# fraunhoferhhi/vvdec

Hardware: NVIDIA H100
Metric: decoded frames/sec, 4K 10-bit Main10 RA, bit-exact YUV vs reference (higher is better)
Workload: dtype int16 samples / int32 accumulate

## Files before the change

### vvdec_b200/csrc/api.cu

```cuda
#include "common.cuh"
#include <stdarg.h>
#include <string.h>
#include <mutex>

namespace b200 {

static thread_local char g_err[512] = "";

void set_error(const char* fmt, ...)
{
  va_list ap; va_start(ap, fmt);
  vsnprintf(g_err, sizeof(g_err), fmt, ap);
  va_end(ap);
}

int ensure_device()
{
  static std::once_flag once;
  static int status = 0;
  std::call_once(once, [] {
    int n = 0;
    if (cudaGetDeviceCount(&n) != cudaSuccess || n == 0) { set_error("no CUDA device: vvdec_b200 has no CPU fallback"); status = B200_ERR_NO_DEVICE; return; }
    int dev = 0; cudaGetDevice(&dev);
    cudaDeviceProp p; cudaGetDeviceProperties(&p, dev);
    if (p.major != 9 || p.minor != 0) { set_error("device %s is sm_%d%d; this library is built for sm_90a only", p.name, p.major, p.minor); status = B200_ERR_NO_DEVICE; }
  });
  if (status) set_error("no usable sm_90 device: vvdec_b200 has no CPU fallback");
  return status;
}

struct HostWrapScratch {
  DevBuf planes[3], tus, coefs, scaling, misc[8];
  cudaStream_t stream = nullptr;
  int init() { if (!stream) { B200_CUDA(cudaStreamCreateWithFlags(&stream, cudaStreamNonBlocking)); } return 0; }
};
static HostWrapScratch g_hw;
HostWrapScratch& host_scratch() { return g_hw; }

static int upload_planes(const b200_geom* g, int16_t* const planes[3], DevPlanes& dp, cudaStream_t s)
{
  const int nPlanes = g->chromaFormat ? 3 : 1;
  for (int c = 0; c < nPlanes; c++) {
    const int ph = c ? g->height >> 1 : g->height;
    const size_t bytes = (size_t)g->stride[c] * ph * sizeof(int16_t);
    if (int rc = g_hw.planes[c].reserve(bytes)) return rc;
    dp.p[c] = g_hw.planes[c].as<int16_t>(); dp.stride[c] = g->stride[c];
    B200_CUDA(cudaMemcpyAsync(dp.p[c], planes[c], bytes, cudaMemcpyHostToDevice, s));
  }
  return 0;
}
static int download_planes(const b200_geom* g, int16_t* const planes[3], const DevPlanes& dp, cudaStream_t s)
{
  const int nPlanes = g->chromaFormat ? 3 : 1;
  for (int c = 0; c < nPlanes; c++) {
    const int ph = c ? g->height >> 1 : g->height;
    B200_CUDA(cudaMemcpyAsync(planes[c], dp.p[c], (size_t)g->stride[c] * ph * sizeof(int16_t), cudaMemcpyDeviceToHost, s));
  }
  return 0;
}

int num_sms()
{
  static int cache[64] = {0};
  int dev = 0; cudaGetDevice(&dev);
  if (dev < 0 || dev >= 64) dev = 0;
  if (!cache[dev]) { int n = 0; if (cudaDeviceGetAttribute(&n, cudaDevAttrMultiProcessorCount, dev) != cudaSuccess || n <= 0) n = 132; cache[dev] = n; }
  return cache[dev];
}

int fetch_list_meta(const int* metaDev, int* cnt, int nLists, const char* what, cudaStream_t s)
{
  int h[LM_INTS];
  B200_CUDA(cudaMemcpyAsync(h, metaDev, sizeof(h), cudaMemcpyDeviceToHost, s));
  B200_CUDA(cudaStreamSynchronize(s));
  for (int i = 0; i < nLists; i++) cnt[i] = h[LM_CNT + i];
  B200_CHECK(!(h[LM_ERR] & 1), "%s: invalid record (reference slots, block size or flag combination)", what);
  B200_CHECK(!(h[LM_ERR] & 2), "%s: more tiles than the picture can hold (overlapping PUs?)", what);
  return 0;
}

}

using namespace b200;

extern "C" {

B200_API const char* b200_last_error(void) { return g_err; }
B200_API const char* b200_version(void) { return "vvdec_b200 0.1 (sm_90a)"; }
B200_API int b200_device_count(void) { int n = 0; return cudaGetDeviceCount(&n) == cudaSuccess ? n : 0; }

B200_API int b200_k1_residual(const b200_geom* g, int16_t* const planes[3], const b200_tu* tus, size_t numTus,
                              const int16_t* coefs, size_t numCoefs, const int32_t* scaling, size_t numScaling, int mode)
{
  B200_CHECK(g && planes && (tus || !numTus), "b200_k1_residual: null argument");
  B200_CHECK(g->bitDepth >= 8 && g->bitDepth <= 12, "b200_k1_residual: bit depth %d unsupported", g->bitDepth);
  if (int rc = ensure_device()) return rc;
  if (int rc = g_hw.init()) return rc;
  cudaStream_t s = g_hw.stream;
  K1Launch L; L.geom = *g; L.numTus = numTus; L.mode = mode;
  if (int rc = upload_planes(g, planes, L.planes, s)) return rc;
  if (int rc = g_hw.tus.reserve(numTus * sizeof(b200_tu))) return rc;
  if (int rc = g_hw.coefs.reserve(numCoefs * sizeof(int16_t) + 16)) return rc;
  if (int rc = g_hw.scaling.reserve(numScaling * sizeof(int32_t) + 16)) return rc;
  if (int rc = g_hw.misc[4].reserve(numTus * 4 + LM_INTS * sizeof(int) + 256)) return rc;
  if (numTus) B200_CUDA(cudaMemcpyAsync(g_hw.tus.p, tus, numTus * sizeof(b200_tu), cudaMemcpyHostToDevice, s));
  if (numCoefs) B200_CUDA(cudaMemcpyAsync(g_hw.coefs.p, coefs, numCoefs * sizeof(int16_t), cudaMemcpyHostToDevice, s));
  if (numScaling) B200_CUDA(cudaMemcpyAsync(g_hw.scaling.p, scaling, numScaling * sizeof(int32_t), cudaMemcpyHostToDevice, s));
  L.tus = g_hw.tus.as<b200_tu>(); L.coefs = g_hw.coefs.as<int16_t>(); L.scaling = g_hw.scaling.as<int32_t>();
  int* meta = g_hw.misc[4].as<int>(); uint32_t* idx = reinterpret_cast<uint32_t*>(meta + LM_INTS);
  if (int rc = launch_tu_bucket(L.tus, numTus, idx, meta, *g, numCoefs, numScaling, s)) return rc;
  L.idx = idx; L.meta = meta;
  if (int rc = fetch_list_meta(meta, L.cnt, K1_LISTS, "b200_k1_residual", s)) return rc;
  StreamSet ss(s);
  if (int rc = launch_k1_residual(L, ss)) return rc;
  if (int rc = download_planes(g, planes, L.planes, s)) return rc;
  B200_CUDA(cudaStreamSynchronize(s));
  return 0;
}

B200_API int b200_lf_deblock(const b200_geom* g, int16_t* const planes[3], const b200_lf_param* lfV, const b200_lf_param* lfH,
                             const uint8_t* ctuSlice, const b200_lf_slice* slices, int numSlices, const b200_lf_seq* seq, int dirs)
{
  B200_CHECK(g && planes && lfV && lfH && slices, "b200_lf_deblock: null argument");
  B200_CHECK(numSlices >= 1 && numSlices <= 64, "b200_lf_deblock: numSlices %d out of range 1..64", numSlices);
  B200_CHECK(g->ctuSize == 32 || g->ctuSize == 64 || g->ctuSize == 128, "b200_lf_deblock: CTU size %d", g->ctuSize);
  if (int rc = ensure_device()) return rc;
  if (int rc = g_hw.init()) return rc;
  cudaStream_t s = g_hw.stream;
  LfLaunch L; L.geom = *g; L.dirs = dirs;
  memset(&L.slices, 0, sizeof(L.slices)); memcpy(L.slices.s, slices, numSlices * sizeof(b200_lf_slice));
  if (seq) L.seq = *seq; else memset(&L.seq, 0, sizeof(L.seq));
  if (int rc = upload_planes(g, planes, L.planes, s)) return rc;
  const size_t n4 = (size_t)((g->width + 3) >> 2) * ((g->height + 3) >> 2);
  const size_t nCtu = (size_t)((g->width + g->ctuSize - 1) / g->ctuSize) * ((g->height + g->ctuSize - 1) / g->ctuSize);
  if (int rc = g_hw.misc[0].reserve(n4 * sizeof(b200_lf_param))) return rc;
  if (int rc = g_hw.misc[1].reserve(n4 * sizeof(b200_lf_param))) return rc;
  if (int rc = g_hw.misc[2].reserve(nCtu)) return rc;
  B200_CUDA(cudaMemcpyAsync(g_hw.misc[0].p, lfV, n4 * sizeof(b200_lf_param), cudaMemcpyHostToDevice, s));
  B200_CUDA(cudaMemcpyAsync(g_hw.misc[1].p, lfH, n4 * sizeof(b200_lf_param), cudaMemcpyHostToDevice, s));
  if (ctuSlice) B200_CUDA(cudaMemcpyAsync(g_hw.misc[2].p, ctuSlice, nCtu, cudaMemcpyHostToDevice, s));
  L.lfV = g_hw.misc[0].as<b200_lf_param>(); L.lfH = g_hw.misc[1].as<b200_lf_param>();
  L.ctuSlice = ctuSlice ? g_hw.misc[2].as<uint8_t>() : nullptr;
  if (int rc = launch_lf_deblock(L, s)) return rc;
  if (int rc = download_planes(g, planes, L.planes, s)) return rc;
  B200_CUDA(cudaStreamSynchronize(s));
  return 0;
}

static int upload_src_alloc_dst(const b200_geom* g, const int16_t* const src[3], DevPlanes& ds, DevPlanes& dd, cudaStream_t s)
{
  const int nPlanes = g->chromaFormat ? 3 : 1;
  for (int c = 0; c < nPlanes; c++) {
    const int ph = c ? g->height >> 1 : g->height;
    const size_t bytes = (size_t)g->stride[c] * ph * sizeof(int16_t);
    if (int rc = g_hw.planes[c].reserve(bytes)) return rc;
    if (int rc = g_hw.misc[3 + c].reserve(bytes)) return rc;
    ds.p[c] = g_hw.planes[c].as<int16_t>(); dd.p[c] = g_hw.misc[3 + c].as<int16_t>(); ds.stride[c] = dd.stride[c] = g->stride[c];
    B200_CUDA(cudaMemcpyAsync(ds.p[c], src[c], bytes, cudaMemcpyHostToDevice, s));
  }
  return 0;
}

B200_API int b200_sao_picture(const b200_geom* g, const int16_t* const src[3], int16_t* const dst[3], const b200_sao_ctu* ctus, const b200_vb* vb)
{
  B200_CHECK(g && src && dst && ctus, "b200_sao_picture: null argument");
  B200_CHECK((g->width & 7) == 0 && (g->stride[0] & 3) == 0 && (!g->chromaFormat || (g->stride[1] & 3) == 0), "b200_sao_picture: width must be a multiple of 8, strides of 4");
  if (int rc = ensure_device()) return rc;
  if (int rc = g_hw.init()) return rc;
  cudaStream_t s = g_hw.stream;
  SaoLaunch L; L.geom = *g;
  if (vb) L.vb = *vb; else memset(&L.vb, 0, sizeof(L.vb));
  if (int rc = upload_src_alloc_dst(g, src, L.src, L.dst, s)) return rc;
  const size_t nCtu = (size_t)((g->width + g->ctuSize - 1) / g->ctuSize) * ((g->height + g->ctuSize - 1) / g->ctuSize);
  if (int rc = g_hw.misc[0].reserve(nCtu * sizeof(b200_sao_ctu))) return rc;
  B200_CUDA(cudaMemcpyAsync(g_hw.misc[0].p, ctus, nCtu * sizeof(b200_sao_ctu), cudaMemcpyHostToDevice, s));
  L.ctus = g_hw.misc[0].as<b200_sao_ctu>();
  if (int rc = launch_sao(L, s)) return rc;
  if (int rc = download_planes(g, dst, L.dst, s)) return rc;
  B200_CUDA(cudaStreamSynchronize(s));
  return 0;
}

B200_API int b200_intra_reconstruct(const b200_geom* g, int16_t* const planes[3], const int16_t* const resi[3], const b200_intra_tu* tus, size_t numTus)
{
  B200_CHECK(g && planes && (tus || !numTus), "b200_intra_reconstruct: null argument");
  B200_CHECK(g->bitDepth >= 8 && g->bitDepth <= 12, "b200_intra_reconstruct: bit depth %d unsupported", g->bitDepth);
  const int nPl = g->chromaFormat ? 3 : 1;
  for (size_t i = 0; i < numTus; i++) {
    const b200_intra_tu& t = tus[i];
    const int w = 1 << t.log2w, h = 1 << t.log2h, pw = t.comp ? g->width >> 1 : g->width, ph = t.comp ? g->height >> 1 : g->height, unit = t.comp ? 2 : 4;
    const bool inCtu = intra_record_in_ctu(t, intra_ctu_log2(*g));
    if (t.flags & B200_INTRA_ISP) {
      B200_CHECK(intra_isp_record_ok(t, i ? &tus[i - 1] : nullptr, g->width, g->height), "b200_intra_reconstruct: record %zu: bad ISP region", i);
      B200_CHECK(inCtu, "b200_intra_reconstruct: intra block record %zu is not inside one CTU", i);
      continue;
    }
    B200_CHECK(t.comp < nPl && t.log2w >= 2 && t.log2w <= 6 && t.log2h >= 1 && t.log2h <= 6 && t.x + w <= pw && t.y + h <= ph && !(t.x % unit) && !(t.y % unit),
               "b200_intra_reconstruct: record %zu: bad geometry", i);
    B200_CHECK(inCtu, "b200_intra_reconstruct: intra block record %zu is not inside one CTU", i);
    B200_CHECK(t.mode <= B200_INTRA_MDLM_T && t.multiRefIdx <= 2 && (!t.multiRefIdx || !t.comp), "b200_intra_reconstruct: record %zu: bad mode / reference line", i);
    B200_CHECK(!t.ciip || (t.ciip <= 3 && t.mode == B200_INTRA_PLANAR), "b200_intra_reconstruct: record %zu: bad CIIP block", i);
    B200_CHECK(t.mode < B200_INTRA_LM || (t.comp && t.log2w <= 5 && t.log2h <= 5 && t.lmAbove <= w && t.lmLeft <= h && (!(t.flags & B200_INTRA_LM_ABOVE) || t.y >= 2) && (!(t.flags & B200_INTRA_LM_LEFT) || t.x >= 2)
                                        && t.x + std::max(w, 2 * (int)t.lmAbove) <= pw && t.y + std::max(h, 2 * (int)t.lmLeft) <= ph), "b200_intra_reconstruct: record %zu: bad CCLM block", i);
    B200_CHECK(t.mode != B200_INTRA_MIP || (!t.comp && !t.multiRefIdx && (t.mip & 0x7f) < ((w == 4 && h == 4) ? 16 : (w == 4 || h == 4 || (w == 8 && h == 8)) ? 8 : 6)),
               "b200_intra_reconstruct: record %zu: bad MIP mode", i);
    B200_CHECK(t.numAbove <= 2 * w / unit && t.numLeft <= 2 * h / unit && (!t.numAbove || t.y > t.multiRefIdx) && (!t.numLeft || t.x > t.multiRefIdx)
               && (!(t.flags & B200_INTRA_AVAIL_TL) || (t.x > t.multiRefIdx && t.y > t.multiRefIdx)) && t.x + (int)t.numAbove * unit <= pw && t.y + (int)t.numLeft * unit <= ph,
               "b200_intra_reconstruct: record %zu: availability outside the picture", i);
  }
  if (int rc = ensure_device()) return rc;
  if (int rc = g_hw.init()) return rc;
  cudaStream_t s = g_hw.stream;
  IntraLaunch L; L.geom = *g; L.numTus = numTus;
  if (int rc = upload_planes(g, planes, L.planes, s)) return rc;
  for (int c = 0; c < 3; c++) {
    L.resi[c] = nullptr; L.owner[c] = nullptr; L.ownerStride[c] = 0; L.ownerBytes[c] = 0;
    if (c >= nPl) continue;
    const int pw = c ? g->width >> 1 : g->width, ph = c ? g->height >> 1 : g->height, unit = c ? 2 : 4;
    L.ownerStride[c] = (pw + unit - 1) / unit; L.ownerBytes[c] = (size_t)L.ownerStride[c] * ((ph + unit - 1) / unit) * sizeof(int);
    if (int rc = g_hw.misc[c].reserve(L.ownerBytes[c])) return rc;
    L.owner[c] = g_hw.misc[c].as<int>();
    if (resi && resi[c]) {
      const size_t bytes = (size_t)g->stride[c] * ph * sizeof(int16_t);
      if (int rc = g_hw.misc[3 + c].reserve(bytes)) return rc;
      B200_CUDA(cudaMemcpyAsync(g_hw.misc[3 + c].p, resi[c], bytes, cudaMemcpyHostToDevice, s));
      L.resi[c] = g_hw.misc[3 + c].as<int16_t>();
    }
  }
  if (int rc = g_hw.tus.reserve(numTus * sizeof(b200_intra_tu) + 16)) return rc;
  if (int rc = g_hw.misc[6].reserve((numTus + 2) * sizeof(int))) return rc;
  if (int rc = g_hw.misc[7].reserve(intra_order_ints(*g, numTus) * sizeof(int))) return rc;
  if (numTus) B200_CUDA(cudaMemcpyAsync(g_hw.tus.p, tus, numTus * sizeof(b200_intra_tu), cudaMemcpyHostToDevice, s));
  L.tus = g_hw.tus.as<b200_intra_tu>(); L.sync = g_hw.misc[6].as<int>(); L.order = g_hw.misc[7].as<int>();
  if (int rc = launch_intra(L, s)) return rc;
  int err = 0;
  if (numTus) B200_CUDA(cudaMemcpyAsync(&err, L.sync + numTus + 1, sizeof(int), cudaMemcpyDeviceToHost, s));
  if (int rc = download_planes(g, planes, L.planes, s)) return rc;
  B200_CUDA(cudaStreamSynchronize(s));
  B200_CHECK(!(err & INTRA_ERR_CTU_BLOCKS), "b200_intra_reconstruct: a CTU holds more than %d intra block records (overlapping records?)", INTRA_MAX_CTU_BLOCKS);
  B200_CHECK(!err, "b200_intra_reconstruct: a block waited for a neighbour that never finished, or the blocks of a CTU are not contiguous (list not in decoding order?)");
  return 0;
}

B200_API int b200_intra_predict(const b200_geom* g, int16_t* const planes[3], const b200_intra_tu* tus, size_t numTus)
{
  return b200_intra_reconstruct(g, planes, nullptr, tus, numTus);
}

B200_API int b200_alf_picture(const b200_geom* g, const int16_t* const src[3], int16_t* const dst[3], const b200_alf_ctu* ctus, const b200_alf_tables* T)
{
  B200_CHECK(g && src && dst && ctus && T, "b200_alf_picture: null argument");
  B200_CHECK((g->width & 7) == 0 && (g->stride[0] & 3) == 0 && (!g->chromaFormat || (g->stride[1] & 3) == 0), "b200_alf_picture: width must be a multiple of 8, strides of 4");
  B200_CHECK(T->numLumaSets >= 16 && T->numLumaSets <= 24, "b200_alf_picture: numLumaSets %d", T->numLumaSets);
  if (int rc = ensure_device()) return rc;
  if (int rc = g_hw.init()) return rc;
  cudaStream_t s = g_hw.stream;
  AlfLaunch L; L.geom = *g;
  if (int rc = upload_src_alloc_dst(g, src, L.src, L.dst, s)) return rc;
  const size_t nCtu = (size_t)((g->width + g->ctuSize - 1) / g->ctuSize) * ((g->height + g->ctuSize - 1) / g->ctuSize);
  const size_t nL = (size_t)T->numLumaSets * 1300, nC = (size_t)T->numChromaAlts * 7, n0 = (size_t)T->numCc[0] * 7, n1 = (size_t)T->numCc[1] * 7;
  const size_t tabElems = 2 * nL + 2 * nC + n0 + n1 + 8;
  if (int rc = g_hw.misc[0].reserve(nCtu * sizeof(b200_alf_ctu))) return rc;
  if (int rc = g_hw.misc[1].reserve(tabElems * sizeof(int16_t))) return rc;
  B200_CUDA(cudaMemcpyAsync(g_hw.misc[0].p, ctus, nCtu * sizeof(b200_alf_ctu), cudaMemcpyHostToDevice, s));
  int16_t* d = g_hw.misc[1].as<int16_t>();
  auto up = [&](const int16_t* h, size_t n, const int16_t*& out) -> int {
    out = d; if (n) B200_CUDA(cudaMemcpyAsync(d, h, n * sizeof(int16_t), cudaMemcpyHostToDevice, s)); d += n; return 0; };
  if (int rc = up(T->lumaCoeff, nL, L.lumaCoeff)) return rc;
  if (int rc = up(T->lumaClip, nL, L.lumaClip)) return rc;
  if (int rc = up(T->chromaCoeff, nC, L.chromaCoeff)) return rc;
  if (int rc = up(T->chromaClip, nC, L.chromaClip)) return rc;
  if (int rc = up(T->ccCoeff[0], n0, L.cc[0])) return rc;
  if (int rc = up(T->ccCoeff[1], n1, L.cc[1])) return rc;
  L.ctus = g_hw.misc[0].as<b200_alf_ctu>();
  StreamSet ss(s);
  if (int rc = launch_alf(L, ss)) return rc;
  if (int rc = download_planes(g, dst, L.dst, s)) return rc;
  B200_CUDA(cudaStreamSynchronize(s));
  return 0;
}

B200_API int b200_mc_predict(const b200_geom* g, int16_t* const dst[3], const int16_t* const* refs, int numSlots,
                             const b200_pu* pus, size_t numPus, int32_t* dmvrMv, size_t numDmvr)
{
  return b200_mc_predict_wp(g, dst, refs, numSlots, pus, numPus, dmvrMv, numDmvr, nullptr, 0);
}

B200_API int b200_mc_predict_wp(const b200_geom* g, int16_t* const dst[3], const int16_t* const* refs, int numSlots,
                                const b200_pu* pus, size_t numPus, int32_t* dmvrMv, size_t numDmvr, const b200_wp* wp, int numWp)
{
  B200_CHECK(g && dst && refs && (pus || !numPus), "b200_mc_predict: null argument");
  B200_CHECK(numSlots >= 1 && numSlots <= B200_MAX_SLOTS, "b200_mc_predict: numSlots %d", numSlots);
  B200_CHECK(numPus < (1u << 26), "b200_mc_predict: too many PUs");
  for (size_t i = 0; i < numPus; i++) {
    B200_CHECK(pus[i].refSlot[0] < numSlots && pus[i].refSlot[1] < numSlots && (pus[i].refSlot[0] >= 0 || pus[i].refSlot[1] >= 0), "b200_mc_predict: PU %zu has invalid reference slots", i);
    B200_CHECK(!((pus[i].flags & B200_PU_DMVR) && g->bitDepth > 10), "b200_mc_predict: DMVR needs bit depth <= 10 (as the reference)");
  }
  if (int rc = ensure_device()) return rc;
  if (int rc = g_hw.init()) return rc;
  cudaStream_t s = g_hw.stream;
  McLaunch L; L.geom = *g;
  if (int rc = upload_planes(g, dst, L.dst, s)) return rc;
  const int nPlanes = g->chromaFormat ? 3 : 1;
  size_t planeBytes[3] = {0, 0, 0}, total = 0;
  for (int c = 0; c < nPlanes; c++) { planeBytes[c] = (((size_t)g->stride[c] * (c ? g->height >> 1 : g->height) * 2) + 255) & ~(size_t)255; total += planeBytes[c]; }
  if (int rc = g_hw.misc[3].reserve(total * numSlots)) return rc;
  std::vector<const int16_t*> ptrs(numSlots * 3, nullptr);
  char* base = g_hw.misc[3].as<char>();
  for (int sl = 0; sl < numSlots; sl++) {
    size_t off = 0;
    for (int c = 0; c < nPlanes; c++) {
      char* d = base + (size_t)sl * total + off;
      B200_CUDA(cudaMemcpyAsync(d, refs[sl * 3 + c], (size_t)g->stride[c] * (c ? g->height >> 1 : g->height) * 2, cudaMemcpyHostToDevice, s));
      ptrs[sl * 3 + c] = reinterpret_cast<const int16_t*>(d); off += planeBytes[c];
    }
  }
  const size_t capTiles = mc_tile_capacity(*g, numPus);
  if (int rc = g_hw.misc[5].reserve(numPus * sizeof(b200_pu) + 64)) return rc;
  if (int rc = g_hw.misc[6].reserve(capTiles * 4 + LM_INTS * sizeof(int) + 256)) return rc;
  if (int rc = g_hw.misc[7].reserve(numDmvr * 8 + 64)) return rc;
  if (numPus) B200_CUDA(cudaMemcpyAsync(g_hw.misc[5].p, pus, numPus * sizeof(b200_pu), cudaMemcpyHostToDevice, s));
  int* meta = g_hw.misc[6].as<int>(); uint32_t* tiles = reinterpret_cast<uint32_t*>(meta + LM_INTS);
  if (int rc = launch_mc_bucket(g_hw.misc[5].as<b200_pu>(), numPus, tiles, capTiles, meta, *g, numSlots, wp ? numWp : 0, numDmvr, s)) return rc;
  L.tiles = tiles; L.meta = meta;
  if (wp && numWp > 0) {
    B200_CHECK(numWp <= 255, "b200_mc_predict_wp: at most 255 weighted-prediction entries");
    if (int rc = g_hw.misc[2].reserve(numWp * sizeof(b200_wp))) return rc;
    B200_CUDA(cudaMemcpyAsync(g_hw.misc[2].p, wp, numWp * sizeof(b200_wp), cudaMemcpyHostToDevice, s));
    L.wp = g_hw.misc[2].as<b200_wp>();
  }
  if (int rc = fetch_list_meta(meta, L.cnt, MC_LISTS, "b200_mc_predict", s)) return rc;
  B200_CUDA(cudaMemsetAsync(g_hw.misc[7].p, 0, numDmvr * 8 + 64, s));
  memset(L.refs, 0, sizeof(L.refs)); for (size_t i = 0; i < ptrs.size(); i++) L.refs[i] = ptrs[i];
  for (int c = 0; c < 3; c++) L.refStride[c] = g->stride[c];
  L.pus = g_hw.misc[5].as<b200_pu>(); L.dmvrMv = dmvrMv ? g_hw.misc[7].as<int32_t>() : nullptr;
  StreamSet ss(s);
  if (int rc = launch_mc(L, ss)) return rc;
  if (int rc = download_planes(g, dst, L.dst, s)) return rc;
  if (dmvrMv && numDmvr) B200_CUDA(cudaMemcpyAsync(dmvrMv, g_hw.misc[7].p, numDmvr * 8, cudaMemcpyDeviceToHost, s));
  B200_CUDA(cudaStreamSynchronize(s));
  return 0;
}

}
```

### vvdec_b200/csrc/common.cuh

```cuda
#pragma once
#include <cuda_runtime.h>
#include <stdint.h>
#include <stdio.h>
#include <string>
#include <vector>
#include <algorithm>
#include "../../include/vvdec_b200.h"

namespace b200 {

void set_error(const char* fmt, ...);

#define B200_CUDA(call)                                                                         \
  do {                                                                                          \
    cudaError_t e_ = (call);                                                                    \
    if (e_ != cudaSuccess) {                                                                    \
      b200::set_error("%s:%d %s -> %s", __FILE__, __LINE__, #call, cudaGetErrorString(e_));     \
      (void)cudaGetLastError();                                                                 \
      return B200_ERR_CUDA;                                                                     \
    }                                                                                           \
  } while (0)

#define B200_CHECK(cond, ...)                                    \
  do {                                                           \
    if (!(cond)) { b200::set_error(__VA_ARGS__); return B200_ERR_PARAM; } \
  } while (0)

__device__ __forceinline__ int clip3(int lo, int hi, int v) { return min(max(v, lo), hi); }
__device__ __forceinline__ int clip16(int v) { return min(max(v, -32768), 32767); }

__device__ __forceinline__ int lmcs_fwd(const b200_lmcs* __restrict__ L, int log2OrgCW, int v, int pmax)
{
  const int idx = v >> log2OrgCW;
  return clip3(0, pmax, (int)__ldg(&L->reshapePivot[idx]) + (((int)__ldg(&L->fwdScaleCoef[idx]) * (v - (int)__ldg(&L->inputPivot[idx])) + (1 << 10)) >> 11));
}
__device__ __forceinline__ int lmcs_scale(int r, int scale, int maxAbs)
{
  r = clip3(-maxAbs - 1, maxAbs, r);
  const int a = abs(r), v = (a * scale + (1 << 10)) >> 11;
  return clip16(r >= 0 ? v : -v);
}

struct DevBuf {
  void*  p   = nullptr;
  size_t cap = 0;
  int reserve(size_t bytes) {
    if (bytes <= cap) return 0;
    if (p) cudaFree(p);
    p = nullptr; cap = 0;
    size_t want = bytes + (bytes >> 2) + 256;
    cudaError_t e = cudaMalloc(&p, want);
    if (e != cudaSuccess) { set_error("cudaMalloc(%zu) -> %s", want, cudaGetErrorString(e)); return B200_ERR_CUDA; }
    cap = want;
    return 0;
  }
  template <class T> T* as() const { return reinterpret_cast<T*>(p); }
  ~DevBuf() { if (p) cudaFree(p); }
};

struct DevPlanes {
  int16_t* p[3] = {nullptr, nullptr, nullptr};
  int      stride[3] = {0, 0, 0};
};

struct KProf { virtual void begin(int family, cudaStream_t s) = 0; virtual void end(int family, cudaStream_t s) = 0; virtual ~KProf() {} };

struct StreamSet {
  cudaStream_t main = nullptr; cudaStream_t aux[4] = {nullptr, nullptr, nullptr, nullptr}; int nAux = 0;
  cudaEvent_t forkEv = nullptr, joinEv[4] = {nullptr, nullptr, nullptr, nullptr};
  bool used[4] = {false, false, false, false};
  StreamSet() {}
  explicit StreamSet(cudaStream_t s) : main(s) {}
  cudaStream_t pick(int i) {
    if (nAux == 0) return main;
    const int k = i % (nAux + 1);
    if (k == nAux) return main;
    if (!used[k]) { cudaEventRecord(forkEv, main); cudaStreamWaitEvent(aux[k], forkEv, 0); used[k] = true; }
    return aux[k];
  }
  void join() { for (int k = 0; k < nAux; k++) if (used[k]) { cudaEventRecord(joinEv[k], aux[k]); cudaStreamWaitEvent(main, joinEv[k], 0); used[k] = false; } }
};

constexpr int MC_LISTS = 17;
constexpr int K1_LISTS = 4;
constexpr int LM_CNT = 0, LM_OFF = 32, LM_CUR = 64, LM_DONE = 96, LM_ERR = 97, LM_INTS = 128;
int launch_mc_bucket(const b200_pu* pus, size_t numPus, uint32_t* tiles, size_t capTiles, int* meta, const b200_geom& g, int numSlots, int numWp, size_t numDmvr, cudaStream_t s);
int launch_tu_bucket(const b200_tu* tus, size_t numTus, uint32_t* idx, int* meta, const b200_geom& g, size_t numCoefs, size_t numScaling, cudaStream_t s);
struct CtuLimits { int numLumaSets, numChromaAlts, numCc[2], numLfSlices; };
int launch_ctu_validate(const b200_sao_ctu* sao, const b200_alf_ctu* alf, const uint8_t* ctuSlice, int nCtu, const CtuLimits& lim, int* meta, cudaStream_t s);
size_t mc_tile_capacity(const b200_geom& g, size_t numPus);
int num_sms();
int fetch_list_meta(const int* metaDev, int* cnt, int nLists, const char* what, cudaStream_t s);

struct K1Launch {
  b200_geom      geom;
  DevPlanes      planes;
  const b200_tu* tus;
  size_t         numTus;
  const uint32_t* idx;
  const int*     meta;
  int            cnt[K1_LISTS];
  const int16_t* coefs;
  const int32_t* scaling;
  int            mode;
  int            compSel = 0;
  const int*     vpduScale = nullptr;
  int16_t*       resi[3] = {nullptr, nullptr, nullptr};
};
int launch_k1_residual(const K1Launch& L, StreamSet& ss, KProf* prof = nullptr);

struct LfSliceTab { b200_lf_slice s[64]; };
struct LfLaunch {
  b200_geom geom; DevPlanes planes;
  const b200_lf_param *lfV, *lfH;
  const uint8_t* ctuSlice;
  LfSliceTab slices; b200_lf_seq seq; int dirs;
};
int launch_lf_deblock(const LfLaunch& L, cudaStream_t s, KProf* prof = nullptr);

struct SaoLaunch { b200_geom geom; DevPlanes src, dst; const b200_sao_ctu* ctus; b200_vb vb; };
int launch_sao(const SaoLaunch& L, cudaStream_t s, KProf* prof = nullptr);

struct AlfLaunch {
  b200_geom geom; DevPlanes src, dst; const b200_alf_ctu* ctus;
  const int16_t *lumaCoeff, *lumaClip, *chromaCoeff, *chromaClip, *cc[2];
};
int launch_alf(const AlfLaunch& L, StreamSet& ss, KProf* prof = nullptr);

constexpr int B200_MAX_SLOTS = 32;
struct McLaunch {
  b200_geom geom; DevPlanes dst;
  const int16_t* refs[B200_MAX_SLOTS * 3];
  int refStride[3];
  const b200_pu* pus;
  const uint32_t* tiles;
  const int* meta;
  int cnt[MC_LISTS];
  int32_t* dmvrMv;
  const b200_wp* wp = nullptr;
  const b200_lmcs* lmcs = nullptr;
  const void* tmaps = nullptr; uint8_t tmapBuf[B200_MAX_SLOTS] = {};
};
int make_mc_tensor_maps(const b200_geom& g, int16_t* const* bufPlanes , int nBufs, void** out);
int launch_mc(const McLaunch& L, StreamSet& ss, KProf* prof = nullptr);
int mc_launch_count(const McLaunch& L);
int k1_launch_count(const K1Launch& L);

struct LmcsLaunch { b200_geom geom; DevPlanes planes; const b200_lmcs* lmcs; const b200_lmcs_vpdu* vpdus; const int16_t* invLut; int* scale; };
int launch_lmcs_vpdu(const LmcsLaunch& L, cudaStream_t s);
int launch_lmcs_inv(const LmcsLaunch& L, cudaStream_t s);

int launch_pack(const DevPlanes& src, const b200_geom& g, int fmt, uint8_t* const dst[3], cudaStream_t s);

struct IntraLaunch { b200_geom geom; DevPlanes planes; const int16_t* resi[3]; const b200_intra_tu* tus; size_t numTus; int* owner[3]; int ownerStride[3]; size_t ownerBytes[3]; int* sync;
                     int* order = nullptr;
                     int compSel = 0;
                   };
inline size_t intra_order_ints(const b200_geom& g, size_t numTus) { return numTus + 8 + 3 * (size_t)((g.width + g.ctuSize - 1) / g.ctuSize) * ((g.height + g.ctuSize - 1) / g.ctuSize); }
inline int intra_ctu_log2(const b200_geom& g) { return g.ctuSize == 128 ? 7 : g.ctuSize == 64 ? 6 : 5; }
__host__ __device__ inline bool intra_record_in_ctu(const b200_intra_tu& t, int ctuLog2)
{
  const int cl = ctuLog2 - (t.comp ? 1 : 0);
  return (t.x >> cl) == ((t.x + (1 << t.log2w) - 1) >> cl) && (t.y >> cl) == ((t.y + (1 << t.log2h) - 1) >> cl);
}
__host__ __device__ inline bool intra_isp_record_ok(const b200_intra_tu& t, const b200_intra_tu* prev, int W, int H)
{
  const int sp = t.mip & 3, k = (t.mip >> 2) & 3, l2n = (t.mip >> 4) & 3, nReg = 1 << l2n, rw = 1 << t.log2w, rh = 1 << t.log2h;
  if (t.comp || t.mode > 66 || t.multiRefIdx || (sp != 1 && sp != 2) || l2n > 2 || (l2n == 0 && (sp != 2 || rw != 4))  || k >= nReg || (t.mip >> 6) || t.log2w < 2 || t.log2w > 6 || t.log2h > 6) return false;
  const int cw = sp == 2 ? rw * nReg : rw, ch = sp == 1 ? rh * nReg : rh, cx = t.x - (sp == 2 ? k * rw : 0), cy = t.y - (sp == 1 ? k * rh : 0);
  if (cw > 64 || ch > 64 || ch < 4 || cw * ch < 32 || cx < 0 || cy < 0 || (cx & 3) || (cy & 3) || cx + cw > W || cy + ch > H) return false;
  if (t.numAbove > 2 * cw / 4 || t.numLeft > 2 * ch / 4 || (t.numAbove && !cy) || (t.numLeft && !cx) || ((t.flags & B200_INTRA_AVAIL_TL) && (!cx || !cy))
      || cx + (int)t.numAbove * 4 > W || cy + (int)t.numLeft * 4 > H || (t.lmLeft && !cx) || (t.lmAbove && !cy)) return false;
  if (k) {
    if (!prev || !(prev->flags & B200_INTRA_ISP) || prev->mip != (uint8_t)(t.mip - 4) || prev->log2w != t.log2w || prev->log2h != t.log2h || prev->mode != t.mode
        || prev->x != t.x - (sp == 2 ? rw : 0) || prev->y != t.y - (sp == 1 ? rh : 0)) return false;
  }
  return true;
}
int launch_intra(const IntraLaunch& L, cudaStream_t s);
int launch_intra_ciip_clear(const b200_intra_tu* tus, size_t numTus, int16_t* const resi[3], const int stride[3], cudaStream_t s);
int launch_intra_validate(const b200_intra_tu* tus, size_t numTus, const b200_geom& g, int* meta, cudaStream_t s);
constexpr int INTRA_ERR_ORDER = 2, INTRA_ERR_CTU_BLOCKS = 4, INTRA_MAX_CTU_BLOCKS = 3072;
int launch_film_grain(const DevPlanes& src, const DevPlanes& dst, const b200_geom& g, const int8_t* pattern, const uint8_t* sLUT, const uint8_t* pLUT,
                      const uint32_t* lineSeeds, uint32_t* seeds, int scaleShift, const uint8_t present[3], cudaStream_t s);
int launch_hash(const DevPlanes& src, const b200_geom& g, int method, uint32_t* acc, uint8_t* digest, cudaStream_t s);

int ensure_device();

}
```

### vvdec_b200/csrc/k5_alf.cu

```cuda
#include "common.cuh"

namespace b200 {

constexpr int TB = 32;
constexpr int HALO = 4;
constexpr int TS = TB + 2 * HALO;
constexpr int TSW = 44;

struct AlfParams {
  const int16_t* src[3]; int16_t* dst[3]; int stride[3];
  int W, H, bitDepth, ctuSize, ctuLog2, ctusW;
  int vecOk;
  int vecOkC;
  const b200_alf_ctu* ctus;
  const int16_t *lumaCoeff, *lumaClip, *chromaCoeff, *chromaClip, *cc0, *cc1;
};

__device__ __forceinline__ void cp_async8(void* smemDst, const void* gmemSrc)
{
  const unsigned d = (unsigned)__cvta_generic_to_shared(smemDst);
  asm volatile("cp.async.ca.shared.global [%0], [%1], 8;\n" :: "r"(d), "l"(gmemSrc));
}

struct AlfExt { int x0, y0, x1, y1, W, H, f, pm; };
__device__ __forceinline__ void alf_map(const AlfExt& E, int& x, int& y)
{
  if ((E.f & B200_ALF_PAD_TL) && x < E.x0 + E.pm && y < E.y0 + E.pm) x = E.x0 + E.pm;
  else if ((E.f & B200_ALF_PAD_BR) && x > E.x1 - E.pm && y > E.y1 - E.pm) x = E.x1 - E.pm;
  x = min(max(x, (E.f & B200_ALF_CLIP_LEFT) ? E.x0 : 0), (E.f & B200_ALF_CLIP_RIGHT) ? E.x1 : E.W - 1);
  y = min(max(y, (E.f & B200_ALF_CLIP_TOP) ? E.y0 : 0), (E.f & B200_ALF_CLIP_BOTTOM) ? E.y1 : E.H - 1);
}

__device__ __forceinline__ int clipd(int c, int ref, int a, int b) { return clip3(-c, c, a - ref) + clip3(-c, c, b - ref); }

__global__ void __launch_bounds__(256) alf_luma_kernel(const AlfParams P)
{
  __shared__ __align__(16) int16_t t[TS][TSW];
  __shared__ uint16_t s_cls[64];
  const int bx0 = blockIdx.x * TB, by0 = blockIdx.y * TB;
  const int tid = threadIdx.x;
  const b200_alf_ctu cp = P.ctus[(by0 >> P.ctuLog2) * P.ctusW + (bx0 >> P.ctuLog2)];
  const int stride = P.stride[0];
  const int bw = min(TB, P.W - bx0), bh = min(TB, P.H - by0);

  if (!(cp.enable[0] & 1)) {
    for (int i = tid; i < bh * (bw >> 2); i += 256) {
      const int y = i / (bw >> 2), x = (i - y * (bw >> 2)) * 4;
      *reinterpret_cast<uint2*>(P.dst[0] + (size_t)(by0 + y) * stride + bx0 + x) = *reinterpret_cast<const uint2*>(P.src[0] + (size_t)(by0 + y) * stride + bx0 + x);
    }
    return;
  }

  const int clipF = cp.enable[0] & ~1;
  if (clipF) {
    AlfExt E; E.x0 = (bx0 >> P.ctuLog2) << P.ctuLog2; E.y0 = (by0 >> P.ctuLog2) << P.ctuLog2; E.x1 = min(E.x0 + P.ctuSize, P.W) - 1; E.y1 = min(E.y0 + P.ctuSize, P.H) - 1;
    E.W = P.W; E.H = P.H; E.f = clipF; E.pm = 0;
    for (int i = tid; i < TS * TS; i += 256) {
      const int ty = i / TS, tx = i - ty * TS;
      int gx = bx0 + tx - HALO, gy = by0 + ty - HALO;
      alf_map(E, gx, gy);
      t[ty][tx] = P.src[0][(size_t)gy * stride + gx];
    }
  } else if (P.vecOk && bx0 >= HALO && bx0 + TB + HALO <= P.W && by0 >= HALO && by0 + TB + HALO <= P.H) {
    const int16_t* s0 = P.src[0] + (size_t)(by0 - HALO) * stride + bx0 - HALO;
    for (int i = tid; i < TS * (TS / 4); i += 256) {
      const int ty = i / (TS / 4), c = i - ty * (TS / 4);
      cp_async8(&t[ty][c * 4], reinterpret_cast<const uint2*>(s0 + (size_t)ty * stride) + c);
    }
    asm volatile("cp.async.wait_all;\n" ::: "memory");
  } else {
    for (int i = tid; i < TS * TS; i += 256) {
      const int ty = i / TS, tx = i - ty * TS;
      const int gx = min(max(bx0 + tx - HALO, 0), P.W - 1), gy = min(max(by0 + ty - HALO, 0), P.H - 1);
      t[ty][tx] = P.src[0][(size_t)gy * stride + gx];
    }
  }
  __syncthreads();

  const int vbH = P.ctuSize, vbPos = P.ctuSize - 4;

  {
    const int b = tid >> 2, r = tid & 3;
    const int bxi = b & 7, byi = b >> 3;
    const int y0 = by0 + byi * 4, x0l = bxi * 4;
    const bool aboveVb = (y0 & (vbH - 1)) == vbPos - 4, belowVb = (y0 & (vbH - 1)) == vbPos;
    int sV = 0, sH = 0, sD0 = 0, sD1 = 0;
    const bool skip = (aboveVb && r == 3) || (belowVb && r == 0);
    if (!skip) {
      const int gy = y0 - 2 + 2 * r;
      const int ly = byi * 4 - 2 + 2 * r + HALO;
      int up = -1, dn2 = 2;
      if (gy > 0 && (gy & (vbH - 1)) == vbPos - 2) dn2 = 1;
      else if (gy > 0 && (gy & (vbH - 1)) == vbPos) up = 0;
#pragma unroll
      for (int c = 0; c < 4; c++) {
        const int lx = x0l - 2 + 2 * c + HALO;
        const int a = t[ly][lx] << 1, bb = t[ly + 1][lx + 1] << 1;
        sV  += abs(a - t[ly + up][lx] - t[ly + 1][lx])          + abs(bb - t[ly][lx + 1] - t[ly + dn2][lx + 1]);
        sH  += abs(a - t[ly][lx + 1] - t[ly][lx - 1])           + abs(bb - t[ly + 1][lx + 2] - t[ly + 1][lx]);
        sD0 += abs(a - t[ly + up][lx - 1] - t[ly + 1][lx + 1])  + abs(bb - t[ly][lx] - t[ly + dn2][lx + 2]);
        sD1 += abs(a - t[ly + 1][lx - 1] - t[ly + up][lx + 1])  + abs(bb - t[ly + dn2][lx] - t[ly][lx + 2]);
      }
    }
#pragma unroll
    for (int m = 1; m < 4; m <<= 1) {
      sV += __shfl_xor_sync(0xffffffffu, sV, m); sH += __shfl_xor_sync(0xffffffffu, sH, m);
      sD0 += __shfl_xor_sync(0xffffffffu, sD0, m); sD1 += __shfl_xor_sync(0xffffffffu, sD1, m);
    }
    if (r == 0) {
      const int shift = P.bitDepth + 4;
      const int act = clip3(0, 15, ((sV + sH) * ((aboveVb || belowVb) ? 96 : 64)) >> shift);
      const unsigned long long TH = 0x4333333332222210ull;
      int classIdx = (int)((TH >> (4 * act)) & 15);
      int hv1, hv0, d1, d0, dirHV, dirD;
      if (sV > sH) { hv1 = sV; hv0 = sH; dirHV = 1; } else { hv1 = sH; hv0 = sV; dirHV = 3; }
      if (sD0 > sD1) { d1 = sD0; d0 = sD1; dirD = 0; } else { d1 = sD1; d0 = sD0; dirD = 2; }
      int hvd1, hvd0, mainDir, secDir;
      if ((unsigned)d1 * (unsigned)hv0 > (unsigned)hv1 * (unsigned)d0) { hvd1 = d1; hvd0 = d0; mainDir = dirD; secDir = dirHV; }
      else { hvd1 = hv1; hvd0 = hv0; mainDir = dirHV; secDir = dirD; }
      int strength = 0;
      if (hvd1 > 2 * hvd0) strength = 1;
      if (hvd1 * 2 > 9 * hvd0) strength = 2;
      if (strength) classIdx += (((mainDir & 1) << 1) + strength) * 5;
      const unsigned TT = 0x31322010u;
      const int tr = (TT >> (4 * (mainDir * 2 + (secDir >> 1)))) & 15;
      s_cls[b] = (uint16_t)(classIdx | (tr << 8));
    }
  }
  __syncthreads();

  {
    const int ry = tid >> 3, rx = (tid & 7) * 4;
    if (ry >= bh || rx >= bw) return;
    const uint16_t k = s_cls[(ry >> 2) * 8 + (rx >> 2)];
    const int off = (k & 0xff) * 13 + (k >> 8) * 13 * 25 + cp.lumaSet * 4 * 25 * 13;
    const int16_t* f = P.lumaCoeff + off; const int16_t* c = P.lumaClip + off;
    int fc[12], cc[12];
#pragma unroll
    for (int i = 0; i < 12; i++) { fc[i] = __ldg(f + i); cc[i] = __ldg(c + i); }
    const int gy = by0 + ry, yVb = gy & (vbH - 1);
    int lim = 3;
    if (yVb < vbPos && yVb >= vbPos - 4) lim = vbPos - 1 - yVb;
    else if (yVb >= vbPos && yVb <= vbPos + 3) lim = yVb - vbPos;
    const bool nearVb = yVb == vbPos - 1 || yVb == vbPos;
    const int r1 = min(1, lim), r2 = min(2, lim), r3 = min(3, lim);
    const int ly = ry + HALO;
    const int pmax = (1 << P.bitDepth) - 1;
    const int lx0 = rx + HALO;
    int out[4];
    bool wide = P.bitDepth > 12;
#pragma unroll
    for (int i = 0; i < 12; i++) wide |= fc[i] != (int)(int8_t)fc[i];
    if (!wide) {
      const uint32_t* R0 = reinterpret_cast<const uint32_t*>(&t[ly][0]) + (lx0 >> 1);
      const uint32_t* P1 = reinterpret_cast<const uint32_t*>(&t[ly + r1][0]) + (lx0 >> 1); const uint32_t* M1 = reinterpret_cast<const uint32_t*>(&t[ly - r1][0]) + (lx0 >> 1);
      const uint32_t* P2 = reinterpret_cast<const uint32_t*>(&t[ly + r2][0]) + (lx0 >> 1); const uint32_t* M2 = reinterpret_cast<const uint32_t*>(&t[ly - r2][0]) + (lx0 >> 1);
      const uint32_t* P3 = reinterpret_cast<const uint32_t*>(&t[ly + r3][0]) + (lx0 >> 1); const uint32_t* M3 = reinterpret_cast<const uint32_t*>(&t[ly - r3][0]) + (lx0 >> 1);
      uint32_t r0w[6], p1w[4], m1w[4], p2w[4], m2w[4], p3w[2], m3w[2];
#pragma unroll
      for (int k = 0; k < 6; k++) r0w[k] = R0[k - 2];
#pragma unroll
      for (int k = 0; k < 4; k++) { p1w[k] = P1[k - 1]; m1w[k] = M1[k - 1]; p2w[k] = P2[k - 1]; m2w[k] = M2[k - 1]; }
#pragma unroll
      for (int k = 0; k < 2; k++) { p3w[k] = P3[k]; m3w[k] = M3[k]; }
      uint32_t r0s[5], p1s[3], m1s[3], p2s[3], m2s[3];
#pragma unroll
      for (int k = 0; k < 5; k++) r0s[k] = __byte_perm(r0w[k], r0w[k + 1], 0x5432);
#pragma unroll
      for (int k = 0; k < 3; k++) {
        p1s[k] = __byte_perm(p1w[k], p1w[k + 1], 0x5432); m1s[k] = __byte_perm(m1w[k], m1w[k + 1], 0x5432);
        p2s[k] = __byte_perm(p2w[k], p2w[k + 1], 0x5432); m2s[k] = __byte_perm(m2w[k], m2w[k + 1], 0x5432);
      }
      int accLo[2] = {0, 0}, accHi[2] = {0, 0};
      uint32_t ncur[2] = {__vneg2(r0w[2]), __vneg2(r0w[3])};
#define R0P(j) (((j) & 1) ? r0s[((j) + 3) >> 1] : r0w[((j) + 4) >> 1])
#define P1P(j) (((j) & 1) ? p1s[((j) + 1) >> 1] : p1w[((j) + 2) >> 1])
#define M1P(j) (((j) & 1) ? m1s[((j) + 1) >> 1] : m1w[((j) + 2) >> 1])
#define P2P(j) (((j) & 1) ? p2s[((j) + 1) >> 1] : p2w[((j) + 2) >> 1])
#define M2P(j) (((j) & 1) ? m2s[((j) + 1) >> 1] : m2w[((j) + 2) >> 1])
#define ALF_TAP(n, A0, B0, A1, B1) { \
        const uint32_t cp = (uint32_t)cc[n] * 0x10001u, cn = __vneg2(cp); const int kl = fc[n] & 0xff, kh = kl << 8; \
        uint32_t d0 = __vmins2(__vmaxs2(__vadd2(A0, ncur[0]), cn), cp), e0 = __vmins2(__vmaxs2(__vadd2(B0, ncur[0]), cn), cp); \
        uint32_t d1 = __vmins2(__vmaxs2(__vadd2(A1, ncur[1]), cn), cp), e1 = __vmins2(__vmaxs2(__vadd2(B1, ncur[1]), cn), cp); \
        d0 = __vadd2(d0, e0); d1 = __vadd2(d1, e1); \
        accLo[0] = __dp2a_lo((int)d0, kl, accLo[0]); accHi[0] = __dp2a_lo((int)d0, kh, accHi[0]); \
        accLo[1] = __dp2a_lo((int)d1, kl, accLo[1]); accHi[1] = __dp2a_lo((int)d1, kh, accHi[1]); }
      ALF_TAP(0,  p3w[0],  m3w[0],  p3w[1],  m3w[1])
      ALF_TAP(1,  P2P(1),  M2P(-1), P2P(3),  M2P(1))
      ALF_TAP(2,  P2P(0),  M2P(0),  P2P(2),  M2P(2))
      ALF_TAP(3,  P2P(-1), M2P(1),  P2P(1),  M2P(3))
      ALF_TAP(4,  P1P(2),  M1P(-2), P1P(4),  M1P(0))
      ALF_TAP(5,  P1P(1),  M1P(-1), P1P(3),  M1P(1))
      ALF_TAP(6,  P1P(0),  M1P(0),  P1P(2),  M1P(2))
      ALF_TAP(7,  P1P(-1), M1P(1),  P1P(1),  M1P(3))
      ALF_TAP(8,  P1P(-2), M1P(2),  P1P(0),  M1P(4))
      ALF_TAP(9,  R0P(3),  R0P(-3), R0P(5),  R0P(-1))
      ALF_TAP(10, R0P(2),  R0P(-2), R0P(4),  R0P(0))
      ALF_TAP(11, R0P(1),  R0P(-1), R0P(3),  R0P(1))
#undef ALF_TAP
#undef R0P
#undef P1P
#undef M1P
#undef P2P
#undef M2P
#pragma unroll
      for (int q = 0; q < 2; q++) {
        const int c0 = (int)(int16_t)(r0w[2 + q] & 0xffff), c1 = (int)r0w[2 + q] >> 16;
        const int s0 = nearVb ? (accLo[q] + 512) >> 10 : (accLo[q] + 64) >> 7, s1 = nearVb ? (accHi[q] + 512) >> 10 : (accHi[q] + 64) >> 7;
        out[2 * q] = clip3(0, pmax, s0 + c0); out[2 * q + 1] = clip3(0, pmax, s1 + c1);
      }
    } else {
    int r0[10], p1[8], m1[8], p2[6], m2[6], p3[4], m3[4];
#pragma unroll
    for (int k = 0; k < 10; k++) r0[k] = t[ly][lx0 - 3 + k];
#pragma unroll
    for (int k = 0; k < 8; k++) { p1[k] = t[ly + r1][lx0 - 2 + k]; m1[k] = t[ly - r1][lx0 - 2 + k]; }
#pragma unroll
    for (int k = 0; k < 6; k++) { p2[k] = t[ly + r2][lx0 - 1 + k]; m2[k] = t[ly - r2][lx0 - 1 + k]; }
#pragma unroll
    for (int k = 0; k < 4; k++) { p3[k] = t[ly + r3][lx0 + k]; m3[k] = t[ly - r3][lx0 + k]; }
#pragma unroll
    for (int i = 0; i < 4; i++) {
      const int cur = r0[i + 3];
      int sum = 0;
      sum += fc[0]  * clipd(cc[0],  cur, p3[i],     m3[i]);
      sum += fc[1]  * clipd(cc[1],  cur, p2[i + 2], m2[i]);
      sum += fc[2]  * clipd(cc[2],  cur, p2[i + 1], m2[i + 1]);
      sum += fc[3]  * clipd(cc[3],  cur, p2[i],     m2[i + 2]);
      sum += fc[4]  * clipd(cc[4],  cur, p1[i + 4], m1[i]);
      sum += fc[5]  * clipd(cc[5],  cur, p1[i + 3], m1[i + 1]);
      sum += fc[6]  * clipd(cc[6],  cur, p1[i + 2], m1[i + 2]);
      sum += fc[7]  * clipd(cc[7],  cur, p1[i + 1], m1[i + 3]);
      sum += fc[8]  * clipd(cc[8],  cur, p1[i],     m1[i + 4]);
      sum += fc[9]  * clipd(cc[9],  cur, r0[i + 6], r0[i]);
      sum += fc[10] * clipd(cc[10], cur, r0[i + 5], r0[i + 1]);
      sum += fc[11] * clipd(cc[11], cur, r0[i + 4], r0[i + 2]);
      sum = nearVb ? (sum + 512) >> 10 : (sum + 64) >> 7;
      out[i] = clip3(0, pmax, sum + cur);
    }
    }
    uint2 o;
    o.x = (unsigned)(out[0] & 0xffff) | ((unsigned)out[1] << 16);
    o.y = (unsigned)(out[2] & 0xffff) | ((unsigned)out[3] << 16);
    *reinterpret_cast<uint2*>(P.dst[0] + (size_t)gy * stride + bx0 + rx) = o;
  }
}

__device__ __forceinline__ void unpack4(const uint2 u, int* d) { d[0] = (int)(int16_t)(u.x & 0xffff); d[1] = (int)u.x >> 16; d[2] = (int)(int16_t)(u.y & 0xffff); d[3] = (int)u.y >> 16; }

__global__ void __launch_bounds__(256) alf_chroma_kernel(const AlfParams P)
{
  const int c = 1 + blockIdx.z;
  const int pw = P.W >> 1, ph = P.H >> 1;
  const int x = (blockIdx.x * 32 + threadIdx.x) * 4, y = blockIdx.y * 8 + threadIdx.y;
  if (x >= pw || y >= ph) return;
  const int l2cs = P.ctuLog2 - 1, cs = 1 << l2cs;
  const b200_alf_ctu cp = P.ctus[(y >> l2cs) * P.ctusW + (x >> l2cs)];
  const int stride = P.stride[c];
  const int16_t* s = P.src[c];
  const int pmax = (1 << P.bitDepth) - 1;
  const int clipF = cp.enable[0] & ~1;
  const bool inner = P.vecOkC && x >= 4 && x + 8 <= pw && !clipF;
  int out[4];
  AlfExt E; E.x0 = (x >> l2cs) << l2cs; E.y0 = (y >> l2cs) << l2cs; E.x1 = min(E.x0 + cs, pw) - 1; E.y1 = min(E.y0 + cs, ph) - 1; E.W = pw; E.H = ph; E.f = clipF;
  E.pm = (cp.enable[c] & B200_ALF_PAD_WIDE) ? 2 : 0;
  auto rowp = [&](int yy) { return s + (size_t)min(max(yy, 0), ph - 1) * stride; };
  auto at = [&](int xx, int yy) { if (clipF) { alf_map(E, xx, yy); return (int)s[(size_t)yy * stride + xx]; } return (int)rowp(yy)[min(max(xx, 0), pw - 1)]; };
  if (cp.enable[c] & 1) {
    const int16_t* f = P.chromaCoeff + cp.chromaAlt[c - 1] * 7; const int16_t* cl = P.chromaClip + cp.chromaAlt[c - 1] * 7;
    int fc[6], cc[6];
#pragma unroll
    for (int i = 0; i < 6; i++) { fc[i] = __ldg(f + i); cc[i] = __ldg(cl + i); }
    const int vbH = cs, vbPos = cs - 2, yVb = y & (vbH - 1);
    int lim = 2;
    if (yVb < vbPos && yVb >= vbPos - 2) lim = vbPos - 1 - yVb;
    else if (yVb >= vbPos && yVb <= vbPos + 1) lim = yVb - vbPos;
    const bool nearVb = yVb == vbPos - 1 || yVb == vbPos;
    const int r1 = min(1, lim), r2 = min(2, lim);
    int r0[8], p1[6], m1[6], p2[4], m2[4];
    if (inner) {
      int t[4];
      const int16_t* q = rowp(y) + x;
      unpack4(__ldg(reinterpret_cast<const uint2*>(q - 4)), t); r0[0] = t[2]; r0[1] = t[3];
      unpack4(__ldg(reinterpret_cast<const uint2*>(q)), r0 + 2);
      unpack4(__ldg(reinterpret_cast<const uint2*>(q + 4)), t); r0[6] = t[0]; r0[7] = t[1];
      q = rowp(y + r1) + x; p1[0] = q[-1]; unpack4(__ldg(reinterpret_cast<const uint2*>(q)), p1 + 1); p1[5] = q[4];
      q = rowp(y - r1) + x; m1[0] = q[-1]; unpack4(__ldg(reinterpret_cast<const uint2*>(q)), m1 + 1); m1[5] = q[4];
      unpack4(__ldg(reinterpret_cast<const uint2*>(rowp(y + r2) + x)), p2);
      unpack4(__ldg(reinterpret_cast<const uint2*>(rowp(y - r2) + x)), m2);
    } else {
#pragma unroll
      for (int k = 0; k < 8; k++) r0[k] = at(x - 2 + k, y);
#pragma unroll
      for (int k = 0; k < 6; k++) { p1[k] = at(x - 1 + k, y + r1); m1[k] = at(x - 1 + k, y - r1); }
#pragma unroll
      for (int k = 0; k < 4; k++) { p2[k] = at(x + k, y + r2); m2[k] = at(x + k, y - r2); }
    }
#pragma unroll
    for (int i = 0; i < 4; i++) {
      const int cur = r0[i + 2];
      int sum = 0;
      sum += fc[0] * clipd(cc[0], cur, p2[i],     m2[i]);
      sum += fc[1] * clipd(cc[1], cur, p1[i + 2], m1[i]);
      sum += fc[2] * clipd(cc[2], cur, p1[i + 1], m1[i + 1]);
      sum += fc[3] * clipd(cc[3], cur, p1[i],     m1[i + 2]);
      sum += fc[4] * clipd(cc[4], cur, r0[i + 4], r0[i]);
      sum += fc[5] * clipd(cc[5], cur, r0[i + 3], r0[i + 1]);
      sum = nearVb ? (sum + 512) >> 10 : (sum + 64) >> 7;
      out[i] = clip3(0, pmax, sum + cur);
    }
  } else {
    unpack4(*reinterpret_cast<const uint2*>(s + (size_t)y * stride + x), out);
  }
  const int ccIdx = cp.ccIdx[c - 1];
  if (ccIdx) {
    const int16_t* f = (c == 1 ? P.cc0 : P.cc1) + (ccIdx - 1) * 7;
    int fc[7];
#pragma unroll
    for (int i = 0; i < 7; i++) fc[i] = __ldg(f + i);
    const int16_t* L = P.src[0]; const int ls = P.stride[0];
    const int ly = y << 1, pos = ly & (P.ctuSize - 1), vbPos = P.ctuSize - 4;
    int o1 = 1, o2 = -1, o3 = 2;
    if (pos == vbPos - 2 || pos == vbPos + 1) o3 = 1;
    else if (pos == vbPos - 1 || pos == vbPos) o1 = o2 = o3 = 0;
    AlfExt EL; EL.x0 = E.x0 << 1; EL.y0 = E.y0 << 1; EL.x1 = min(EL.x0 + P.ctuSize, P.W) - 1; EL.y1 = min(EL.y0 + P.ctuSize, P.H) - 1; EL.W = P.W; EL.H = P.H; EL.f = clipF; EL.pm = 0;
    auto lrow = [&](int yy) { return L + (size_t)min(max(yy, 0), P.H - 1) * ls; };
    auto lat = [&](int xx, int yy) { if (clipF) { alf_map(EL, xx, yy); return (int)L[(size_t)yy * ls + xx]; } return (int)lrow(yy)[min(max(xx, 0), P.W - 1)]; };
    const int half = (1 << P.bitDepth) >> 1;
    int a[9], bb[9], up[4], dn[4];
    if (inner) {
      int t[4];
      const int16_t* q = lrow(ly) + 2 * x;
      a[0] = q[-1]; unpack4(__ldg(reinterpret_cast<const uint2*>(q)), a + 1); unpack4(__ldg(reinterpret_cast<const uint2*>(q + 4)), a + 5);
      q = lrow(ly + o1) + 2 * x;
      bb[0] = q[-1]; unpack4(__ldg(reinterpret_cast<const uint2*>(q)), bb + 1); unpack4(__ldg(reinterpret_cast<const uint2*>(q + 4)), bb + 5);
      q = lrow(ly + o2) + 2 * x;
      unpack4(__ldg(reinterpret_cast<const uint2*>(q)), t); up[0] = t[0]; up[1] = t[2]; unpack4(__ldg(reinterpret_cast<const uint2*>(q + 4)), t); up[2] = t[0]; up[3] = t[2];
      q = lrow(ly + o3) + 2 * x;
      unpack4(__ldg(reinterpret_cast<const uint2*>(q)), t); dn[0] = t[0]; dn[1] = t[2]; unpack4(__ldg(reinterpret_cast<const uint2*>(q + 4)), t); dn[2] = t[0]; dn[3] = t[2];
    } else {
#pragma unroll
      for (int k = 0; k < 9; k++) { a[k] = lat(2 * x - 1 + k, ly); bb[k] = lat(2 * x - 1 + k, ly + o1); }
#pragma unroll
      for (int i = 0; i < 4; i++) { up[i] = lat(2 * (x + i), ly + o2); dn[i] = lat(2 * (x + i), ly + o3); }
    }
#pragma unroll
    for (int i = 0; i < 4; i++) {
      const int cur = a[2 * i + 1];
      int sum = fc[0] * (up[i] - cur) + fc[1] * (a[2 * i] - cur) + fc[2] * (a[2 * i + 2] - cur)
              + fc[3] * (bb[2 * i] - cur) + fc[4] * (bb[2 * i + 1] - cur) + fc[5] * (bb[2 * i + 2] - cur)
              + fc[6] * (dn[i] - cur);
      sum = (sum + 64) >> 7;
      sum = clip3(0, pmax, sum + half) - half;
      out[i] = clip3(0, pmax, sum + out[i]);
    }
  }
  uint2 o;
  o.x = (unsigned)(out[0] & 0xffff) | ((unsigned)out[1] << 16);
  o.y = (unsigned)(out[2] & 0xffff) | ((unsigned)out[3] << 16);
  *reinterpret_cast<uint2*>(P.dst[c] + (size_t)y * stride + x) = o;
}

int launch_alf(const AlfLaunch& L, StreamSet& ss, KProf* prof)
{
  cudaStream_t s = ss.main;
  AlfParams P;
  for (int c = 0; c < 3; c++) { P.src[c] = L.src.p[c]; P.dst[c] = L.dst.p[c]; P.stride[c] = L.src.stride[c]; }
  P.W = L.geom.width; P.H = L.geom.height; P.bitDepth = L.geom.bitDepth; P.ctuSize = L.geom.ctuSize;
  P.ctuLog2 = P.ctuSize == 128 ? 7 : P.ctuSize == 64 ? 6 : 5; P.ctusW = (P.W + P.ctuSize - 1) / P.ctuSize;
  P.ctus = L.ctus; P.lumaCoeff = L.lumaCoeff; P.lumaClip = L.lumaClip; P.chromaCoeff = L.chromaCoeff; P.chromaClip = L.chromaClip;
  P.cc0 = L.cc[0]; P.cc1 = L.cc[1];
  P.vecOk = (P.stride[0] & 3) == 0 && (reinterpret_cast<uintptr_t>(P.src[0]) & 7) == 0;
  P.vecOkC = P.vecOk && (P.stride[1] & 3) == 0 && (P.stride[2] & 3) == 0 && (reinterpret_cast<uintptr_t>(P.src[1]) & 7) == 0 && (reinterpret_cast<uintptr_t>(P.src[2]) & 7) == 0;
  dim3 grdL((P.W + TB - 1) / TB, (P.H + TB - 1) / TB);
  if (L.geom.chromaFormat == 1) {
    cudaStream_t sc = ss.pick(0);
    dim3 blk(32, 8), grd(((P.W >> 1) / 4 + 31) / 32, ((P.H >> 1) + 7) / 8, 2);
    if (prof) prof->begin(B200_KF_ALF_CHROMA, sc);
    alf_chroma_kernel<<<grd, blk, 0, sc>>>(P);
    B200_CUDA(cudaGetLastError());
    if (prof) prof->end(B200_KF_ALF_CHROMA, sc);
  }
  if (prof) prof->begin(B200_KF_ALF_LUMA, s);
  alf_luma_kernel<<<grdL, 256, 0, s>>>(P);
  B200_CUDA(cudaGetLastError());
  if (prof) prof->end(B200_KF_ALF_LUMA, s);
  ss.join();
  return 0;
}

}
```

### vvdec_b200/csrc/picture.cu

```cuda
#include "common.cuh"
#include <string.h>
#include <vector>

namespace b200 {

static inline size_t align256(size_t v) { return (v + 255) & ~(size_t)255; }

struct Arena {
  DevBuf buf;
  const b200_pu* pus = nullptr; size_t numPus = 0; const uint32_t* tiles = nullptr; int* mcMeta = nullptr;
  int* hMeta = nullptr;
  const b200_tu* tus = nullptr; size_t numTus = 0; const uint32_t* tuIdx = nullptr; int* tuMeta = nullptr; const int16_t* coefs = nullptr; const int32_t* scaling = nullptr;
  const b200_lf_param *lfV = nullptr, *lfH = nullptr; const uint8_t* ctuSlice = nullptr; LfSliceTab lfSlices; b200_lf_seq lfSeq;
  const b200_sao_ctu* sao = nullptr; b200_vb vb;
  const b200_alf_ctu* alf = nullptr; const int16_t *lumaCoeff = nullptr, *lumaClip = nullptr, *chromaCoeff = nullptr, *chromaClip = nullptr, *cc[2] = {nullptr, nullptr};
  int32_t* dmvrMv = nullptr; size_t numDmvr = 0;
  const b200_wp* wp = nullptr;
  const b200_lmcs* lmcs = nullptr; const int16_t* lmcsInv = nullptr; const b200_lmcs_vpdu* lmcsVpdus = nullptr; int* lmcsScale = nullptr; bool lmcsChromaAdj = false;
  int16_t* given[3] = {nullptr, nullptr, nullptr};
  const b200_intra_tu* intraTus = nullptr; size_t numIntraTus = 0; int* intraOwner[3] = {nullptr, nullptr, nullptr}; int intraOwnerStride[3] = {0, 0, 0}; size_t intraOwnerBytes[3] = {0, 0, 0}; int* intraSync = nullptr; int* intraOrder = nullptr;
  int dstSlot = 0, flags = 0;
  bool ciipResi = false;
  bool valid = false;
  cudaEvent_t uploaded = nullptr, done = nullptr; bool donePending = false;
};

}

using namespace b200;

struct CtxProf : b200::KProf {
  struct Rec { int family; cudaEvent_t a, b; };
  std::vector<Rec> recs; std::vector<cudaEvent_t> pool; Rec cur{};
  cudaEvent_t get() { cudaEvent_t e; if (!pool.empty()) { e = pool.back(); pool.pop_back(); } else cudaEventCreate(&e); return e; }
  void begin(int f, cudaStream_t s) override { cur.family = f; cur.a = get(); cur.b = get(); cudaEventRecord(cur.a, s); }
  void end(int, cudaStream_t s) override { cudaEventRecord(cur.b, s); recs.push_back(cur); }
};

struct b200_ctx {
  b200_geom g;
  CtxProf prof; bool profiling = false;
  int numSlots = 0, numArenas = 0, device = 0;
  cudaStream_t stream = nullptr, copyStream = nullptr, upStream = nullptr;
  StreamSet ss;
  cudaEvent_t ev[2] = {nullptr, nullptr};
  std::vector<cudaEvent_t> readDone; std::vector<char> readPending;
  cudaEvent_t ticketEv[16]; cudaEvent_t finalEv = nullptr; int nextTicket = 0;
  DevBuf outStage[2]; int nextStage = 0;
  size_t planeBytes[3] = {0, 0, 0}, picBytes = 0;
  std::vector<int16_t*> bufs;
  std::vector<int> slotBuf;
  int work[2] = {0, 0};
  std::vector<Arena> arenas;
  int nextArena = 0;
  long long launches = 0;
  DevBuf grainStage[2], grainTab;
  DevBuf resiBuf;
  DevBuf hashBuf;
  void* tmaps = nullptr;

  DevPlanes planes(int buf) const {
    DevPlanes d; char* b = reinterpret_cast<char*>(bufs[buf]);
    d.p[0] = reinterpret_cast<int16_t*>(b); d.p[1] = reinterpret_cast<int16_t*>(b + planeBytes[0]); d.p[2] = reinterpret_cast<int16_t*>(b + planeBytes[0] + planeBytes[1]);
    for (int c = 0; c < 3; c++) d.stride[c] = g.stride[c];
    return d;
  }
};

extern "C" {

B200_API int b200_ctx_create(b200_ctx** out, const b200_geom* g, int numSlots, int numArenas, int device)
{
  B200_CHECK(out && g, "b200_ctx_create: null argument");
  B200_CHECK(numSlots >= 1 && numSlots <= B200_MAX_SLOTS && numArenas >= 1 && numArenas <= 256, "b200_ctx_create: numSlots %d / numArenas %d out of range", numSlots, numArenas);
  B200_CHECK((g->width & 7) == 0 && (g->height & 7) == 0, "b200_ctx_create: picture size must be a multiple of 8");
  B200_CHECK(g->chromaFormat == 0 || g->chromaFormat == 1, "b200_ctx_create: only 4:0:0 and 4:2:0");
  B200_CHECK(g->ctuSize == 32 || g->ctuSize == 64 || g->ctuSize == 128, "b200_ctx_create: CTU size %d", g->ctuSize);
  if (int rc = ensure_device()) return rc;
  if (device >= 0) B200_CUDA(cudaSetDevice(device));
  b200_ctx* c = new b200_ctx;
  c->g = *g; c->numSlots = numSlots; c->numArenas = numArenas;
  B200_CUDA(cudaGetDevice(&c->device));
  B200_CUDA(cudaStreamCreateWithFlags(&c->stream, cudaStreamNonBlocking));
  B200_CUDA(cudaStreamCreateWithFlags(&c->copyStream, cudaStreamNonBlocking));
  B200_CUDA(cudaStreamCreateWithFlags(&c->upStream, cudaStreamNonBlocking));
  c->ss.main = c->stream; c->ss.nAux = 3;
  B200_CUDA(cudaEventCreateWithFlags(&c->ss.forkEv, cudaEventDisableTiming));
  for (int k = 0; k < c->ss.nAux; k++) { B200_CUDA(cudaStreamCreateWithFlags(&c->ss.aux[k], cudaStreamNonBlocking)); B200_CUDA(cudaEventCreateWithFlags(&c->ss.joinEv[k], cudaEventDisableTiming)); }
  B200_CUDA(cudaEventCreate(&c->ev[0])); B200_CUDA(cudaEventCreate(&c->ev[1]));
  B200_CUDA(cudaEventCreateWithFlags(&c->finalEv, cudaEventDisableTiming));
  for (auto& e : c->ticketEv) B200_CUDA(cudaEventCreateWithFlags(&e, cudaEventDisableTiming));
  for (int k = 0; k < 3; k++) c->planeBytes[k] = (k == 0 || g->chromaFormat) ? align256((size_t)g->stride[k] * (k ? g->height >> 1 : g->height) * 2) : 0;
  c->picBytes = c->planeBytes[0] + c->planeBytes[1] + c->planeBytes[2];
  c->bufs.resize(numSlots + 2); c->slotBuf.resize(numSlots);
  c->readDone.resize(numSlots + 2); c->readPending.assign(numSlots + 2, 0);
  for (auto& e : c->readDone) B200_CUDA(cudaEventCreateWithFlags(&e, cudaEventDisableTiming));
  for (int i = 0; i < numSlots + 2; i++) { B200_CUDA(cudaMalloc(&c->bufs[i], c->picBytes)); B200_CUDA(cudaMemset(c->bufs[i], 0, c->picBytes)); }
  for (int s = 0; s < numSlots; s++) c->slotBuf[s] = s;
  {
    std::vector<int16_t*> pl;
    for (int i = 0; i < numSlots + 2; i++) { DevPlanes d = c->planes(i); for (int k = 0; k < 3; k++) pl.push_back(d.p[k]); }
    if (int rc = make_mc_tensor_maps(*g, pl.data(), numSlots + 2, &c->tmaps)) return rc;
  }
  c->work[0] = numSlots; c->work[1] = numSlots + 1;
  c->arenas.resize(numArenas);
  for (auto& A : c->arenas) { B200_CUDA(cudaEventCreateWithFlags(&A.uploaded, cudaEventDisableTiming)); B200_CUDA(cudaEventCreateWithFlags(&A.done, cudaEventDisableTiming)); B200_CUDA(cudaHostAlloc(reinterpret_cast<void**>(&A.hMeta), (2 * LM_INTS + 4) * sizeof(int), cudaHostAllocDefault)); }
  *out = c;
  return 0;
}

B200_API void b200_ctx_destroy(b200_ctx* c)
{
  if (!c) return;
  cudaStreamSynchronize(c->stream); cudaStreamSynchronize(c->copyStream); cudaStreamSynchronize(c->upStream);
  for (auto& A : c->arenas) { cudaEventDestroy(A.uploaded); cudaEventDestroy(A.done); if (A.hMeta) cudaFreeHost(A.hMeta); }
  cudaStreamDestroy(c->upStream);
  for (auto p : c->bufs) cudaFree(p);
  if (c->tmaps) cudaFree(c->tmaps);
  for (auto e : c->readDone) cudaEventDestroy(e);
  for (auto e : c->ticketEv) cudaEventDestroy(e);
  cudaEventDestroy(c->finalEv); cudaStreamDestroy(c->copyStream);
  for (int k = 0; k < c->ss.nAux; k++) { cudaStreamSynchronize(c->ss.aux[k]); cudaStreamDestroy(c->ss.aux[k]); cudaEventDestroy(c->ss.joinEv[k]); }
  cudaEventDestroy(c->ss.forkEv);
  cudaEventDestroy(c->ev[0]); cudaEventDestroy(c->ev[1]);
  cudaStreamDestroy(c->stream);
  delete c;
}

B200_API int b200_ctx_load_slot(b200_ctx* c, int slot, const int16_t* const planes[3])
{
  B200_CHECK(c && planes && slot >= 0 && slot < c->numSlots, "b200_ctx_load_slot: bad argument");
  DevPlanes d = c->planes(c->slotBuf[slot]);
  for (int k = 0; k < (c->g.chromaFormat ? 3 : 1); k++)
    B200_CUDA(cudaMemcpyAsync(d.p[k], planes[k], (size_t)c->g.stride[k] * (k ? c->g.height >> 1 : c->g.height) * 2, cudaMemcpyHostToDevice, c->stream));
  B200_CUDA(cudaStreamSynchronize(c->stream));
  return 0;
}

B200_API int b200_pic_upload(b200_ctx* c, const b200_picture* p)
{
  B200_CHECK(c && p, "b200_pic_upload: null argument");
  B200_CHECK(p->dstSlot >= 0 && p->dstSlot < c->numSlots, "b200_pic_upload: dstSlot %d", p->dstSlot);
  B200_CHECK(!(p->flags & B200_PIC_DEBLOCK) || (p->lfV && p->lfH && p->lfSlices && p->numLfSlices >= 1 && p->numLfSlices <= 64), "b200_pic_upload: deblocking data missing");
  B200_CHECK(!(p->flags & B200_PIC_SAO) || p->sao, "b200_pic_upload: SAO data missing");
  B200_CHECK(!(p->flags & B200_PIC_ALF) || (p->alf && p->alfTabs && p->alfTabs->numLumaSets >= 16), "b200_pic_upload: ALF data missing");
  B200_CHECK(p->numPus < (1u << 26) && p->numTus < (1u << 31), "b200_pic_upload: too many records");
  B200_CHECK(p->numWp >= 0 && p->numWp <= 255 && (p->wp || !p->numWp), "b200_pic_upload: weighted-prediction table (at most 255 entries)");
  B200_CHECK(!(p->flags & B200_PIC_LMCS) || (p->lmcs && p->lmcs->invLUT && (!p->lmcs->chromaAdj || p->lmcs->vpdus) && p->lmcs->orgCW == (1 << c->g.bitDepth) / 16), "b200_pic_upload: LMCS data missing or inconsistent");
  B200_CHECK(!p->numIntraTus || (p->intraTus && p->numIntraTus < (1u << 30)), "b200_pic_upload: intra list missing");
  B200_CUDA(cudaSetDevice(c->device));
  const int ai = c->nextArena; c->nextArena = (c->nextArena + 1) % c->numArenas;
  Arena& A = c->arenas[ai];
  A.valid = false;
  const b200_geom& g = c->g;
  const size_t n4 = (size_t)((g.width + 3) >> 2) * ((g.height + 3) >> 2);
  const size_t nCtu = (size_t)((g.width + g.ctuSize - 1) / g.ctuSize) * ((g.height + g.ctuSize - 1) / g.ctuSize);
  const size_t capTiles = mc_tile_capacity(g, 0);
  const b200_alf_tables* T = p->alfTabs;
  const size_t nL = (p->flags & B200_PIC_ALF) ? (size_t)T->numLumaSets * 1300 : 0, nC = (p->flags & B200_PIC_ALF) ? (size_t)T->numChromaAlts * 7 : 0;
  const size_t n0 = (p->flags & B200_PIC_ALF) ? (size_t)T->numCc[0] * 7 : 0, n1 = (p->flags & B200_PIC_ALF) ? (size_t)T->numCc[1] * 7 : 0;
  size_t off = 0;
  auto take = [&](size_t bytes) { size_t o = off; off += align256(bytes + 16); return o; };
  const size_t oPus = take(p->numPus * sizeof(b200_pu)), oT = take(capTiles * 4), oMeta = take(2 * LM_INTS * sizeof(int)), oIdx = take(p->numTus * 4);
  const size_t oTus = take(p->numTus * sizeof(b200_tu)), oCoef = take(p->numCoefs * 2), oScal = take(p->numScaling * 4);
  const size_t oLfV = take((p->flags & B200_PIC_DEBLOCK) ? n4 * 6 : 0), oLfH = take((p->flags & B200_PIC_DEBLOCK) ? n4 * 6 : 0), oCs = take(nCtu);
  const size_t oSao = take((p->flags & B200_PIC_SAO) ? nCtu * sizeof(b200_sao_ctu) : 0);
  const size_t oAlf = take((p->flags & B200_PIC_ALF) ? nCtu * sizeof(b200_alf_ctu) : 0), oTab = take((2 * nL + 2 * nC + n0 + n1) * 2);
  const size_t oDm = take(p->numDmvr * 8);
  const size_t oWp = take((size_t)p->numWp * sizeof(b200_wp));
  const bool lm = p->flags & B200_PIC_LMCS;
  const int vs = g.ctuSize == 128 ? 64 : g.ctuSize; const size_t nVpdu = (size_t)((g.width + vs - 1) / vs) * ((g.height + vs - 1) / vs);
  const size_t oLm = take(lm ? sizeof(b200_lmcs) : 0), oLmLut = take(lm ? sizeof(int16_t) << g.bitDepth : 0), oLmVp = take(lm ? nVpdu * sizeof(b200_lmcs_vpdu) : 0), oLmSc = take(lm ? nVpdu * sizeof(int) : 0);
  const bool hasGiven = p->given[0] != nullptr;
  const size_t oGiven = take(hasGiven ? c->picBytes : 0);
  size_t oOwn[3] = {0, 0, 0}, ownBytes[3] = {0, 0, 0}; int ownStride[3] = {0, 0, 0};
  const size_t oIntra = take(p->numIntraTus * sizeof(b200_intra_tu)), oSync = take(p->numIntraTus ? (p->numIntraTus + 2) * sizeof(int) : 0), oOrder = take(p->numIntraTus ? intra_order_ints(g, p->numIntraTus) * sizeof(int) : 0);
  for (int k = 0; k < (g.chromaFormat ? 3 : 1) && p->numIntraTus; k++) {
    const int pw = k ? g.width >> 1 : g.width, ph = k ? g.height >> 1 : g.height, unit = k ? 2 : 4;
    ownStride[k] = (pw + unit - 1) / unit; ownBytes[k] = (size_t)ownStride[k] * ((ph + unit - 1) / unit) * sizeof(int); oOwn[k] = take(ownBytes[k]);
  }
  if (p->numIntraTus) if (int rc = c->resiBuf.reserve(c->picBytes)) return rc;
  if (off > A.buf.cap) { B200_CUDA(cudaStreamSynchronize(c->stream)); B200_CUDA(cudaStreamSynchronize(c->upStream)); A.donePending = false; }
  if (int rc = A.buf.reserve(off)) return rc;
  char* base = A.buf.as<char>();
  cudaStream_t s = c->upStream;
  if (A.donePending) { B200_CUDA(cudaStreamWaitEvent(s, A.done, 0)); A.donePending = false; }
  auto h2d = [&](size_t o, const void* src, size_t bytes) -> int { if (bytes) B200_CUDA(cudaMemcpyAsync(base + o, src, bytes, cudaMemcpyHostToDevice, s)); return 0; };
  if (int rc = h2d(oPus, p->pus, p->numPus * sizeof(b200_pu))) return rc;
  if (int rc = h2d(oTus, p->tus, p->numTus * sizeof(b200_tu))) return rc;
  if (int rc = h2d(oCoef, p->coefs, p->numCoefs * 2)) return rc;
  if (int rc = h2d(oScal, p->scaling, p->numScaling * 4)) return rc;
  if (p->flags & B200_PIC_DEBLOCK) {
    if (int rc = h2d(oLfV, p->lfV, n4 * 6)) return rc;
    if (int rc = h2d(oLfH, p->lfH, n4 * 6)) return rc;
    if (p->ctuSlice) if (int rc = h2d(oCs, p->ctuSlice, nCtu)) return rc;
    memset(&A.lfSlices, 0, sizeof(A.lfSlices)); memcpy(A.lfSlices.s, p->lfSlices, p->numLfSlices * sizeof(b200_lf_slice));
    if (p->lfSeq) A.lfSeq = *p->lfSeq; else memset(&A.lfSeq, 0, sizeof(A.lfSeq));
  }
  if (p->flags & B200_PIC_SAO) { if (int rc = h2d(oSao, p->sao, nCtu * sizeof(b200_sao_ctu))) return rc; if (p->vb) A.vb = *p->vb; else memset(&A.vb, 0, sizeof(A.vb)); }
  if (p->flags & B200_PIC_ALF) {
    if (int rc = h2d(oAlf, p->alf, nCtu * sizeof(b200_alf_ctu))) return rc;
    size_t o = oTab;
    auto up = [&](const int16_t* src, size_t n, const int16_t*& view) -> int { view = reinterpret_cast<const int16_t*>(base + o); int rc = h2d(o, src, n * 2); o += n * 2; return rc; };
    if (int rc = up(T->lumaCoeff, nL, A.lumaCoeff)) return rc;
    if (int rc = up(T->lumaClip, nL, A.lumaClip)) return rc;
    if (int rc = up(T->chromaCoeff, nC, A.chromaCoeff)) return rc;
    if (int rc = up(T->chromaClip, nC, A.chromaClip)) return rc;
    if (int rc = up(T->ccCoeff[0], n0, A.cc[0])) return rc;
    if (int rc = up(T->ccCoeff[1], n1, A.cc[1])) return rc;
  }
  if (int rc = h2d(oWp, p->wp, (size_t)p->numWp * sizeof(b200_wp))) return rc;
  A.wp = p->numWp ? reinterpret_cast<const b200_wp*>(base + oWp) : nullptr;
  if (lm) {
    if (int rc = h2d(oLm, p->lmcs, sizeof(b200_lmcs))) return rc;
    if (int rc = h2d(oLmLut, p->lmcs->invLUT, sizeof(int16_t) << g.bitDepth)) return rc;
    if (p->lmcs->chromaAdj) if (int rc = h2d(oLmVp, p->lmcs->vpdus, nVpdu * sizeof(b200_lmcs_vpdu))) return rc;
    A.lmcs = reinterpret_cast<const b200_lmcs*>(base + oLm); A.lmcsInv = reinterpret_cast<const int16_t*>(base + oLmLut);
    A.lmcsVpdus = reinterpret_cast<const b200_lmcs_vpdu*>(base + oLmVp); A.lmcsScale = reinterpret_cast<int*>(base + oLmSc); A.lmcsChromaAdj = p->lmcs->chromaAdj != 0;
  } else { A.lmcs = nullptr; A.lmcsChromaAdj = false; }
  if (hasGiven) {
    size_t o = oGiven;
    for (int k = 0; k < (g.chromaFormat ? 3 : 1); k++) {
      A.given[k] = reinterpret_cast<int16_t*>(base + o);
      if (int rc = h2d(o, p->given[k], (size_t)g.stride[k] * (k ? g.height >> 1 : g.height) * 2)) return rc;
      o += c->planeBytes[k];
    }
  } else A.given[0] = A.given[1] = A.given[2] = nullptr;
  A.pus = reinterpret_cast<const b200_pu*>(base + oPus); A.numPus = p->numPus;
  A.tus = reinterpret_cast<const b200_tu*>(base + oTus); A.numTus = p->numTus;
  A.coefs = reinterpret_cast<const int16_t*>(base + oCoef); A.scaling = reinterpret_cast<const int32_t*>(base + oScal);
  A.lfV = reinterpret_cast<const b200_lf_param*>(base + oLfV); A.lfH = reinterpret_cast<const b200_lf_param*>(base + oLfH);
  A.ctuSlice = p->ctuSlice ? reinterpret_cast<const uint8_t*>(base + oCs) : nullptr;
  A.sao = reinterpret_cast<const b200_sao_ctu*>(base + oSao); A.alf = reinterpret_cast<const b200_alf_ctu*>(base + oAlf);
  A.dmvrMv = p->numDmvr ? reinterpret_cast<int32_t*>(base + oDm) : nullptr; A.numDmvr = p->numDmvr;
  if (p->numDmvr) B200_CUDA(cudaMemsetAsync(base + oDm, 0, p->numDmvr * 8, s));
  if (int rc = h2d(oIntra, p->intraTus, p->numIntraTus * sizeof(b200_intra_tu))) return rc;
  A.intraTus = reinterpret_cast<const b200_intra_tu*>(base + oIntra); A.numIntraTus = p->numIntraTus; A.intraSync = reinterpret_cast<int*>(base + oSync); A.intraOrder = reinterpret_cast<int*>(base + oOrder);
  for (int k = 0; k < 3; k++) { A.intraOwner[k] = ownBytes[k] ? reinterpret_cast<int*>(base + oOwn[k]) : nullptr; A.intraOwnerStride[k] = ownStride[k]; A.intraOwnerBytes[k] = ownBytes[k]; }
  A.ciipResi = false;
  for (size_t i = 0; i < p->numIntraTus && !A.ciipResi; i++) { const b200_intra_tu& t = p->intraTus[i]; A.ciipResi = t.ciip && !(t.flags & B200_INTRA_ISP) && (t.flags & B200_INTRA_ADD_RESI); }
  A.dstSlot = p->dstSlot; A.flags = p->flags; A.valid = true;
  A.mcMeta = reinterpret_cast<int*>(base + oMeta); A.tuMeta = A.mcMeta + LM_INTS;
  if (int rc = launch_mc_bucket(reinterpret_cast<const b200_pu*>(base + oPus), p->numPus, reinterpret_cast<uint32_t*>(base + oT), capTiles, A.mcMeta, g, c->numSlots, p->numWp, p->numDmvr, s)) return rc;
  if (int rc = launch_tu_bucket(reinterpret_cast<const b200_tu*>(base + oTus), p->numTus, reinterpret_cast<uint32_t*>(base + oIdx), A.tuMeta, g, p->numCoefs, p->numScaling, s)) return rc;
  A.tiles = reinterpret_cast<const uint32_t*>(base + oT); A.tuIdx = reinterpret_cast<const uint32_t*>(base + oIdx);
  c->launches += 4;
  {
    CtuLimits lim; const bool alfOn = p->flags & B200_PIC_ALF;
    lim.numLumaSets = alfOn ? T->numLumaSets : 0; lim.numChromaAlts = alfOn ? T->numChromaAlts : 0; lim.numCc[0] = alfOn ? T->numCc[0] : 0; lim.numCc[1] = alfOn ? T->numCc[1] : 0;
    lim.numLfSlices = p->numLfSlices;
    const bool any = (p->flags & (B200_PIC_SAO | B200_PIC_ALF)) || ((p->flags & B200_PIC_DEBLOCK) && p->ctuSlice);
    if (int rc = launch_ctu_validate((p->flags & B200_PIC_SAO) ? A.sao : nullptr, alfOn ? A.alf : nullptr, (p->flags & B200_PIC_DEBLOCK) ? A.ctuSlice : nullptr, (int)nCtu, lim, A.mcMeta, s)) return rc;
    if (any) c->launches += 1;
  }
  if (A.numIntraTus) { if (int rc = launch_intra_validate(A.intraTus, A.numIntraTus, g, A.mcMeta, s)) return rc; c->launches += 1; }
  B200_CUDA(cudaMemcpyAsync(A.hMeta, A.mcMeta, 2 * LM_INTS * sizeof(int), cudaMemcpyDeviceToHost, s));
  B200_CUDA(cudaEventRecord(A.uploaded, s));
  return ai;
}

B200_API int b200_pic_run(b200_ctx* c, int ai)
{
  B200_CHECK(c && ai >= 0 && ai < c->numArenas && c->arenas[ai].valid, "b200_pic_run: bad arena %d", ai);
  B200_CUDA(cudaSetDevice(c->device));
  Arena& A = c->arenas[ai];
  cudaStream_t s = c->stream;
  B200_CUDA(cudaEventSynchronize(A.uploaded));
  B200_CHECK(!(A.hMeta[LM_ERR] & 1), "b200_pic_run: the picture's PU list holds an invalid record (reference slots, block size or flag combination)");
  B200_CHECK(!(A.hMeta[LM_ERR] & 2), "b200_pic_run: more MC tiles than the picture can hold (overlapping PUs?)");
  B200_CHECK(!(A.hMeta[LM_ERR] & 8), "b200_pic_run: an intra block record is invalid (geometry, mode, or availability reaching outside the picture)");
  B200_CHECK(!(A.hMeta[LM_ERR] & 4), "b200_pic_run: a CTU record (SAO type / band, ALF filter index, slice index) is out of range");
  B200_CHECK(!A.hMeta[LM_INTS + LM_ERR], "b200_pic_run: the picture's TU list holds an invalid record");
  B200_CUDA(cudaStreamWaitEvent(s, A.uploaded, 0));
  const b200_geom& g = c->g;
  int cur = c->work[0], other = c->work[1];
  for (int b : {cur, other}) if (c->readPending[b]) { B200_CUDA(cudaStreamWaitEvent(s, c->readDone[b], 0)); c->readPending[b] = 0; }
  DevPlanes P = c->planes(cur);
  if (A.given[0]) {
    for (int k = 0; k < (g.chromaFormat ? 3 : 1); k++)
      B200_CUDA(cudaMemcpyAsync(P.p[k], A.given[k], (size_t)g.stride[k] * (k ? g.height >> 1 : g.height) * 2, cudaMemcpyDeviceToDevice, s));
  }
  if (A.numPus) {
    McLaunch L; L.geom = g; L.dst = P; memset(L.refs, 0, sizeof(L.refs));
    for (int sl = 0; sl < c->numSlots; sl++) { DevPlanes d = c->planes(c->slotBuf[sl]); for (int k = 0; k < 3; k++) L.refs[sl * 3 + k] = d.p[k]; }
    for (int k = 0; k < 3; k++) L.refStride[k] = g.stride[k];
    L.tmaps = c->tmaps; for (int sl = 0; sl < c->numSlots; sl++) L.tmapBuf[sl] = (uint8_t)c->slotBuf[sl];
    L.pus = A.pus; L.tiles = A.tiles; L.meta = A.mcMeta; L.dmvrMv = A.dmvrMv; L.lmcs = A.lmcs; L.wp = A.wp;
    for (int l = 0; l < MC_LISTS; l++) L.cnt[l] = A.hMeta[LM_CNT + l];
    if (int rc = launch_mc(L, c->ss, c->profiling ? &c->prof : nullptr)) return rc;
    c->launches += mc_launch_count(L);
  }
  LmcsLaunch LM; LM.geom = g; LM.planes = P; LM.lmcs = A.lmcs; LM.vpdus = A.lmcsVpdus; LM.invLut = A.lmcsInv; LM.scale = A.lmcsScale;
  const bool twoPass = A.lmcs && A.lmcsChromaAdj;
  A.hMeta[2 * LM_INTS] = 0;
  int16_t* resiPl[3] = {nullptr, nullptr, nullptr};
  if (A.numIntraTus) {
    uint8_t* rb = c->resiBuf.as<uint8_t>(); resiPl[0] = reinterpret_cast<int16_t*>(rb); resiPl[1] = reinterpret_cast<int16_t*>(rb + c->planeBytes[0]); resiPl[2] = reinterpret_cast<int16_t*>(rb + c->planeBytes[0] + c->planeBytes[1]);
    if (A.ciipResi) { if (int rc = launch_intra_ciip_clear(A.intraTus, A.numIntraTus, resiPl, P.stride, s)) return rc; c->launches += 1; }
  }
  auto runK1 = [&](int compSel, const int* vpduScale) -> int {
    if (!A.numTus) return 0;
    K1Launch L; L.geom = g; L.planes = P; L.tus = A.tus; L.numTus = A.numTus; L.idx = A.tuIdx; L.meta = A.tuMeta; L.coefs = A.coefs; L.scaling = A.scaling; L.mode = 0;
    for (int k = 0; k < 3; k++) L.resi[k] = resiPl[k];
    for (int l = 0; l < K1_LISTS; l++) L.cnt[l] = A.hMeta[LM_INTS + LM_CNT + l];
    L.compSel = compSel; L.vpduScale = vpduScale;
    if (int rc = launch_k1_residual(L, c->ss, c->profiling ? &c->prof : nullptr)) return rc;
    c->launches += k1_launch_count(L);
    return 0;
  };
  auto runK6 = [&](int compSel) -> int {
    if (!A.numIntraTus) return 0;
    IntraLaunch L; L.geom = g; L.planes = P; L.tus = A.intraTus; L.numTus = A.numIntraTus; L.sync = A.intraSync; L.order = A.intraOrder; L.compSel = compSel;
    for (int k = 0; k < 3; k++) { L.resi[k] = resiPl[k]; L.owner[k] = A.intraOwner[k]; L.ownerStride[k] = A.intraOwnerStride[k]; L.ownerBytes[k] = A.intraOwnerBytes[k]; }
    if (c->profiling) c->prof.begin(B200_KF_INTRA, s);
    if (int rc = launch_intra(L, s)) return rc;
    if (c->profiling) c->prof.end(B200_KF_INTRA, s);
    c->launches += compSel == 2 ? 1 : 5;
    return 0;
  };
  if (twoPass) {
    if (int rc = runK1(1, nullptr)) return rc;
    if (int rc = runK6(1)) return rc;
    if (c->profiling) c->prof.begin(B200_KF_LMCS, s);
    if (int rc = launch_lmcs_vpdu(LM, s)) return rc;
    if (c->profiling) c->prof.end(B200_KF_LMCS, s);
    c->launches += 1;
    if (int rc = runK1(2, A.lmcsScale)) return rc;
    if (int rc = runK6(2)) return rc;
  } else {
    if (int rc = runK1(0, nullptr)) return rc;
    if (int rc = runK6(0)) return rc;
  }
  if (A.numIntraTus) B200_CUDA(cudaMemcpyAsync(A.hMeta + 2 * LM_INTS, A.intraSync + A.numIntraTus + 1, sizeof(int), cudaMemcpyDeviceToHost, s));
  if (A.lmcs) { if (c->profiling) c->prof.begin(B200_KF_LMCS, s); if (int rc = launch_lmcs_inv(LM, s)) return rc; if (c->profiling) c->prof.end(B200_KF_LMCS, s); c->launches += 1; }
  if (A.flags & B200_PIC_DEBLOCK) {
    LfLaunch L; L.geom = g; L.planes = P; L.lfV = A.lfV; L.lfH = A.lfH; L.ctuSlice = A.ctuSlice; L.slices = A.lfSlices; L.seq = A.lfSeq; L.dirs = 3;
    if (int rc = launch_lf_deblock(L, s, c->profiling ? &c->prof : nullptr)) return rc;
    c->launches += 2;
  }
  if (A.flags & B200_PIC_SAO) {
    SaoLaunch L; L.geom = g; L.src = P; L.dst = c->planes(other); L.ctus = A.sao; L.vb = A.vb;
    if (int rc = launch_sao(L, s, c->profiling ? &c->prof : nullptr)) return rc;
    c->launches += 1;
    std::swap(cur, other); P = c->planes(cur);
  }
  if (A.flags & B200_PIC_ALF) {
    AlfLaunch L; L.geom = g; L.src = P; L.dst = c->planes(other); L.ctus = A.alf;
    L.lumaCoeff = A.lumaCoeff; L.lumaClip = A.lumaClip; L.chromaCoeff = A.chromaCoeff; L.chromaClip = A.chromaClip; L.cc[0] = A.cc[0]; L.cc[1] = A.cc[1];
    if (int rc = launch_alf(L, c->ss, c->profiling ? &c->prof : nullptr)) return rc;
    c->launches += g.chromaFormat ? 2 : 1;
    std::swap(cur, other);
  }
  B200_CUDA(cudaEventRecord(A.done, s)); A.donePending = true;
  const int old = c->slotBuf[A.dstSlot];
  c->slotBuf[A.dstSlot] = cur;
  c->work[0] = old; c->work[1] = other;
  return 0;
}

B200_API int b200_decompress_picture(b200_ctx* c, const b200_picture* p)
{
  const int ai = b200_pic_upload(c, p);
  if (ai < 0) return ai;
  if (int rc = b200_pic_run(c, ai)) return rc;
  return ai;
}

B200_API int b200_wait_picture(b200_ctx* c, int ai, int32_t* dmvrMv, size_t numDmvr)
{
  B200_CHECK(c, "b200_wait_picture: null context");
  if (dmvrMv && ai >= 0 && ai < c->numArenas && c->arenas[ai].dmvrMv) {
    const size_t n = numDmvr < c->arenas[ai].numDmvr ? numDmvr : c->arenas[ai].numDmvr;
    B200_CUDA(cudaMemcpyAsync(dmvrMv, c->arenas[ai].dmvrMv, n * 8, cudaMemcpyDeviceToHost, c->stream));
  }
  B200_CUDA(cudaStreamSynchronize(c->upStream));
  B200_CUDA(cudaStreamSynchronize(c->stream));
  if (ai >= 0 && ai < c->numArenas && c->arenas[ai].numIntraTus) {
    const int err = c->arenas[ai].hMeta[2 * LM_INTS];
    B200_CHECK(!(err & INTRA_ERR_CTU_BLOCKS), "b200_wait_picture: a CTU holds more than %d intra block records (overlapping records?)", INTRA_MAX_CTU_BLOCKS);
    B200_CHECK(!err, "b200_wait_picture: an intra block waited for a neighbour that never finished (intra list not in decoding order?)");
  }
  return 0;
}

B200_API int b200_get_frame(b200_ctx* c, int slot, int16_t* const planes[3])
{
  B200_CHECK(c && planes && slot >= 0 && slot < c->numSlots, "b200_get_frame: bad argument");
  DevPlanes d = c->planes(c->slotBuf[slot]);
  for (int k = 0; k < (c->g.chromaFormat ? 3 : 1); k++)
    B200_CUDA(cudaMemcpyAsync(planes[k], d.p[k], (size_t)c->g.stride[k] * (k ? c->g.height >> 1 : c->g.height) * 2, cudaMemcpyDeviceToHost, c->stream));
  B200_CUDA(cudaStreamSynchronize(c->stream));
  return 0;
}

static int copy2d_host(void* dst, size_t dpitch, const void* src, size_t spitch, size_t wBytes, size_t h, cudaMemcpyKind kind, cudaStream_t s)
{
  const cudaError_t e = cudaMemcpy2DAsync(dst, dpitch, src, spitch, wBytes, h, kind, s);
  if (e != cudaErrorInvalidValue) { B200_CUDA(e); return 0; }
  (void)cudaGetLastError();
  void* stage = nullptr;
  B200_CUDA(cudaMallocHost(&stage, wBytes * h));
  int rc = 0;
  if (kind == cudaMemcpyHostToDevice) {
    for (size_t y = 0; y < h; y++) memcpy((char*)stage + y * wBytes, (const char*)src + y * spitch, wBytes);
    const cudaError_t e2 = cudaMemcpy2DAsync(dst, dpitch, stage, wBytes, wBytes, h, kind, s);
    const cudaError_t e3 = e2 == cudaSuccess ? cudaStreamSynchronize(s) : e2;
    if (e3 != cudaSuccess) { set_error("copy2d_host: staged H2D copy -> %s", cudaGetErrorString(e3)); (void)cudaGetLastError(); rc = B200_ERR_CUDA; }
  } else {
    const cudaError_t e2 = cudaMemcpy2DAsync(stage, wBytes, src, spitch, wBytes, h, kind, s);
    const cudaError_t e3 = e2 == cudaSuccess ? cudaStreamSynchronize(s) : e2;
    if (e3 != cudaSuccess) { set_error("copy2d_host: staged D2H copy -> %s", cudaGetErrorString(e3)); (void)cudaGetLastError(); rc = B200_ERR_CUDA; }
    else for (size_t y = 0; y < h; y++) memcpy((char*)dst + y * dpitch, (const char*)stage + y * wBytes, wBytes);
  }
  cudaFreeHost(stage);
  return rc;
}

B200_API int b200_ctx_load_slot_strided(b200_ctx* c, int slot, const int16_t* const planes[3], const ptrdiff_t strides[3])
{
  B200_CHECK(c && planes && strides && slot >= 0 && slot < c->numSlots, "b200_ctx_load_slot_strided: bad argument");
  DevPlanes d = c->planes(c->slotBuf[slot]);
  for (int k = 0; k < (c->g.chromaFormat ? 3 : 1); k++) {
    const size_t w = k ? c->g.width >> 1 : c->g.width, h = k ? c->g.height >> 1 : c->g.height;
    B200_CHECK(planes[k] && strides[k] >= (ptrdiff_t)w, "b200_ctx_load_slot_strided: plane %d", k);
    if (int rc = copy2d_host(d.p[k], (size_t)c->g.stride[k] * 2, planes[k], (size_t)strides[k] * 2, w * 2, h, cudaMemcpyHostToDevice, c->stream)) return rc;
  }
  B200_CUDA(cudaStreamSynchronize(c->stream));
  return 0;
}

B200_API int b200_get_frame_strided(b200_ctx* c, int slot, int16_t* const planes[3], const ptrdiff_t strides[3])
{
  B200_CHECK(c && planes && strides && slot >= 0 && slot < c->numSlots, "b200_get_frame_strided: bad argument");
  DevPlanes d = c->planes(c->slotBuf[slot]);
  for (int k = 0; k < (c->g.chromaFormat ? 3 : 1); k++) {
    const size_t w = k ? c->g.width >> 1 : c->g.width, h = k ? c->g.height >> 1 : c->g.height;
    B200_CHECK(planes[k] && strides[k] >= (ptrdiff_t)w, "b200_get_frame_strided: plane %d", k);
    if (int rc = copy2d_host(planes[k], (size_t)strides[k] * 2, d.p[k], (size_t)c->g.stride[k] * 2, w * 2, h, cudaMemcpyDeviceToHost, c->stream)) return rc;
  }
  B200_CUDA(cudaStreamSynchronize(c->stream));
  return 0;
}

B200_API int b200_get_frame_async(b200_ctx* c, int slot, int16_t* const planes[3])
{
  B200_CHECK(c && planes && slot >= 0 && slot < c->numSlots, "b200_get_frame_async: bad argument");
  const int buf = c->slotBuf[slot];
  DevPlanes d = c->planes(buf);
  B200_CUDA(cudaEventRecord(c->finalEv, c->stream));
  B200_CUDA(cudaStreamWaitEvent(c->copyStream, c->finalEv, 0));
  for (int k = 0; k < (c->g.chromaFormat ? 3 : 1); k++)
    B200_CUDA(cudaMemcpyAsync(planes[k], d.p[k], (size_t)c->g.stride[k] * (k ? c->g.height >> 1 : c->g.height) * 2, cudaMemcpyDeviceToHost, c->copyStream));
  B200_CUDA(cudaEventRecord(c->readDone[buf], c->copyStream)); c->readPending[buf] = 1;
  const int t = c->nextTicket; c->nextTicket = (c->nextTicket + 1) & 15;
  B200_CUDA(cudaEventRecord(c->ticketEv[t], c->copyStream));
  return t;
}

B200_API int b200_get_frame_device_async(b200_ctx* c, int slot, int16_t* const planesDev[3], void* cudaStream)
{
  B200_CHECK(c && planesDev && slot >= 0 && slot < c->numSlots, "b200_get_frame_device_async: bad argument");
  cudaStream_t st = static_cast<cudaStream_t>(cudaStream);
  const int buf = c->slotBuf[slot];
  DevPlanes d = c->planes(buf);
  B200_CUDA(cudaEventRecord(c->finalEv, c->stream));
  B200_CUDA(cudaStreamWaitEvent(st, c->finalEv, 0));
  for (int k = 0; k < (c->g.chromaFormat ? 3 : 1); k++) {
    B200_CHECK(planesDev[k], "b200_get_frame_device_async: plane %d", k);
    B200_CUDA(cudaMemcpyAsync(planesDev[k], d.p[k], (size_t)c->g.stride[k] * (k ? c->g.height >> 1 : c->g.height) * 2, cudaMemcpyDeviceToDevice, st));
  }
  B200_CUDA(cudaEventRecord(c->readDone[buf], st)); c->readPending[buf] = 1;
  return 0;
}

B200_API size_t b200_frame_bytes(const b200_geom* g, int fmt, int comp)
{
  if (!g || comp < 0 || comp > 2 || (comp && !g->chromaFormat)) return 0;
  const size_t W = comp ? g->width >> 1 : g->width, H = comp ? g->height >> 1 : g->height;
  if (fmt == B200_OUT_PYUV) return W / 4 * 5 * H;
  if (fmt == B200_OUT_8) return W * H;
  return (size_t)g->stride[comp] * H * 2;
}

B200_API int b200_get_frame_fmt_async(b200_ctx* c, int slot, int fmt, void* const planes[3])
{
  B200_CHECK(c && planes && slot >= 0 && slot < c->numSlots, "b200_get_frame_fmt_async: bad argument");
  if (fmt == B200_OUT_16) { int16_t* const p16[3] = {(int16_t*)planes[0], (int16_t*)planes[1], (int16_t*)planes[2]}; return b200_get_frame_async(c, slot, p16); }
  B200_CHECK(fmt == B200_OUT_PYUV || fmt == B200_OUT_8, "b200_get_frame_fmt_async: unknown format %d", fmt);
  if (fmt == B200_OUT_PYUV && (c->g.bitDepth != 10 || (c->g.width & 7))) { set_error("b200_get_frame_fmt_async: pyuv needs 10 bit and a width divisible by 8 (as vvdecapp)"); return B200_ERR_UNSUPPORTED; }
  B200_CUDA(cudaSetDevice(c->device));
  const int nPl = c->g.chromaFormat ? 3 : 1;
  size_t bytes[3] = {0, 0, 0}, off[3] = {0, 0, 0}, total = 0;
  for (int k = 0; k < nPl; k++) { bytes[k] = b200_frame_bytes(&c->g, fmt, k); off[k] = total; total += (bytes[k] + 255) & ~(size_t)255; }
  const int st = c->nextStage; c->nextStage ^= 1;
  if (total > c->outStage[st].cap) B200_CUDA(cudaStreamSynchronize(c->copyStream));
  if (int rc = c->outStage[st].reserve(total)) return rc;
  const int buf = c->slotBuf[slot];
  DevPlanes d = c->planes(buf);
  B200_CUDA(cudaEventRecord(c->finalEv, c->stream));
  B200_CUDA(cudaStreamWaitEvent(c->copyStream, c->finalEv, 0));
  uint8_t* dst[3]; for (int k = 0; k < 3; k++) dst[k] = c->outStage[st].as<uint8_t>() + off[k];
  if (int rc = launch_pack(d, c->g, fmt, dst, c->copyStream)) return rc;
  c->launches += nPl;
  B200_CUDA(cudaEventRecord(c->readDone[buf], c->copyStream)); c->readPending[buf] = 1;
  for (int k = 0; k < nPl; k++) B200_CUDA(cudaMemcpyAsync(planes[k], dst[k], bytes[k], cudaMemcpyDeviceToHost, c->copyStream));
  const int t = c->nextTicket; c->nextTicket = (c->nextTicket + 1) & 15;
  B200_CUDA(cudaEventRecord(c->ticketEv[t], c->copyStream));
  return t;
}

B200_API int b200_get_frame_grain_async(b200_ctx* c, int slot, int fmt, void* const planes[3], const b200_film_grain* fg)
{
  B200_CHECK(c && planes && fg && slot >= 0 && slot < c->numSlots, "b200_get_frame_grain_async: bad argument");
  B200_CHECK(fg->pattern && fg->sLUT && fg->pLUT && fg->lineSeeds, "b200_get_frame_grain_async: table missing");
  B200_CHECK(fmt == B200_OUT_16 || fmt == B200_OUT_PYUV || fmt == B200_OUT_8, "b200_get_frame_grain_async: unknown format %d", fmt);
  const b200_geom& g = c->g;
  if (g.bitDepth != 8 && g.bitDepth != 10) { set_error("b200_get_frame_grain_async: film grain needs 8 or 10 bit (FilmGrainImpl::set_depth)"); return B200_ERR_UNSUPPORTED; }
  if (fmt == B200_OUT_PYUV && (g.bitDepth != 10 || (g.width & 7))) { set_error("b200_get_frame_grain_async: pyuv needs 10 bit and a width divisible by 8 (as vvdecapp)"); return B200_ERR_UNSUPPORTED; }
  const int bs = g.bitDepth - 8;
  B200_CHECK(fg->scaleShift + bs >= 8 && fg->scaleShift + bs <= 13, "b200_get_frame_grain_async: scaleShift %d out of range (FilmGrainImpl.cpp:142)", fg->scaleShift);
  B200_CHECK(g.width > 128, "b200_get_frame_grain_async: width must exceed 128 (FilmGrainImpl.cpp:140)");
  for (int k = 0; k < 768; k++) B200_CHECK((fg->pLUT[k] >> 4) < 8, "b200_get_frame_grain_async: pLUT[%d] selects pattern %d (only 8 exist)", k, fg->pLUT[k] >> 4);
  B200_CUDA(cudaSetDevice(c->device));
  const int nPl = g.chromaFormat ? 3 : 1, nbx = (g.width + 15) / 16, nby = (g.height + 15) / 16;
  const int st = c->nextStage; c->nextStage ^= 1;
  const size_t oS = 2 * 8 * 4096, oP = oS + 768, oL = oP + 768, oB = oL + (size_t)nby * 4, tabBytes = oB + (size_t)nbx * nby * 4;
  if (tabBytes > c->grainTab.cap || c->picBytes > c->grainStage[st].cap) B200_CUDA(cudaStreamSynchronize(c->copyStream));
  if (int rc = c->grainTab.reserve(tabBytes)) return rc;
  if (int rc = c->grainStage[st].reserve(c->picBytes)) return rc;
  uint8_t* tb = c->grainTab.as<uint8_t>();
  B200_CUDA(cudaMemcpyAsync(tb, fg->pattern, oS, cudaMemcpyHostToDevice, c->copyStream));
  B200_CUDA(cudaMemcpyAsync(tb + oS, fg->sLUT, 768, cudaMemcpyHostToDevice, c->copyStream));
  B200_CUDA(cudaMemcpyAsync(tb + oP, fg->pLUT, 768, cudaMemcpyHostToDevice, c->copyStream));
  B200_CUDA(cudaMemcpyAsync(tb + oL, fg->lineSeeds, (size_t)nby * 4, cudaMemcpyHostToDevice, c->copyStream));
  const int buf = c->slotBuf[slot];
  DevPlanes src = c->planes(buf), gr = src;
  { uint8_t* b = c->grainStage[st].as<uint8_t>(); gr.p[0] = reinterpret_cast<int16_t*>(b); gr.p[1] = reinterpret_cast<int16_t*>(b + c->planeBytes[0]); gr.p[2] = reinterpret_cast<int16_t*>(b + c->planeBytes[0] + c->planeBytes[1]); }
  B200_CUDA(cudaEventRecord(c->finalEv, c->stream));
  B200_CUDA(cudaStreamWaitEvent(c->copyStream, c->finalEv, 0));
  if (int rc = launch_film_grain(src, gr, g, reinterpret_cast<const int8_t*>(tb), tb + oS, tb + oP, reinterpret_cast<const uint32_t*>(tb + oL),
                                 reinterpret_cast<uint32_t*>(tb + oB), fg->scaleShift, fg->compPresent, c->copyStream)) return rc;
  c->launches += 1 + nPl;
  B200_CUDA(cudaEventRecord(c->readDone[buf], c->copyStream)); c->readPending[buf] = 1;
  if (fmt == B200_OUT_16) {
    for (int k = 0; k < nPl; k++) B200_CUDA(cudaMemcpyAsync(planes[k], gr.p[k], (size_t)g.stride[k] * (k ? g.height >> 1 : g.height) * 2, cudaMemcpyDeviceToHost, c->copyStream));
  } else {
    size_t bytes[3] = {0, 0, 0}, off[3] = {0, 0, 0}, total = 0;
    for (int k = 0; k < nPl; k++) { bytes[k] = b200_frame_bytes(&g, fmt, k); off[k] = total; total += (bytes[k] + 255) & ~(size_t)255; }
    if (total > c->outStage[st].cap) B200_CUDA(cudaStreamSynchronize(c->copyStream));
    if (int rc = c->outStage[st].reserve(total)) return rc;
    uint8_t* dst[3]; for (int k = 0; k < 3; k++) dst[k] = c->outStage[st].as<uint8_t>() + off[k];
    if (int rc = launch_pack(gr, g, fmt, dst, c->copyStream)) return rc;
    c->launches += nPl;
    for (int k = 0; k < nPl; k++) B200_CUDA(cudaMemcpyAsync(planes[k], dst[k], bytes[k], cudaMemcpyDeviceToHost, c->copyStream));
  }
  const int t = c->nextTicket; c->nextTicket = (c->nextTicket + 1) & 15;
  B200_CUDA(cudaEventRecord(c->ticketEv[t], c->copyStream));
  return t;
}

B200_API int b200_frame_hash_async(b200_ctx* c, int slot, int method, uint8_t* digest)
{
  B200_CHECK(c && digest && slot >= 0 && slot < c->numSlots, "b200_frame_hash_async: bad argument");
  if (method == B200_HASH_MD5) { set_error("b200_frame_hash_async: MD5 is a serial chain over each plane and is not computed on the device; use CRC or checksum"); return B200_ERR_UNSUPPORTED; }
  B200_CHECK(method == B200_HASH_CRC || method == B200_HASH_CHECKSUM, "b200_frame_hash_async: unknown method %d", method);
  B200_CUDA(cudaSetDevice(c->device));
  if (int rc = c->hashBuf.reserve(16 * 32)) return rc;
  const int t = c->nextTicket; c->nextTicket = (c->nextTicket + 1) & 15;
  uint32_t* acc = c->hashBuf.as<uint32_t>() + t * 8; uint8_t* dig = reinterpret_cast<uint8_t*>(acc + 4);
  const int buf = c->slotBuf[slot];
  B200_CUDA(cudaEventRecord(c->finalEv, c->stream));
  B200_CUDA(cudaStreamWaitEvent(c->copyStream, c->finalEv, 0));
  B200_CUDA(cudaMemsetAsync(acc, 0, 32, c->copyStream));
  if (int rc = launch_hash(c->planes(buf), c->g, method, acc, dig, c->copyStream)) return rc;
  c->launches += (c->g.chromaFormat ? 3 : 1) + 1;
  B200_CUDA(cudaEventRecord(c->readDone[buf], c->copyStream)); c->readPending[buf] = 1;
  B200_CUDA(cudaMemcpyAsync(digest, dig, 12, cudaMemcpyDeviceToHost, c->copyStream));
  B200_CUDA(cudaEventRecord(c->ticketEv[t], c->copyStream));
  return t;
}

B200_API int b200_frame_wait(b200_ctx* c, int ticket)
{
  B200_CHECK(c && ticket >= 0 && ticket < 16, "b200_frame_wait: bad ticket");
  B200_CUDA(cudaEventSynchronize(c->ticketEv[ticket]));
  return 0;
}

B200_API int b200_ctx_mark(b200_ctx* c, int which) { B200_CHECK(c && (which == 0 || which == 1), "b200_ctx_mark"); B200_CUDA(cudaEventRecord(c->ev[which], c->stream)); return 0; }
B200_API int b200_ctx_elapsed_ms(b200_ctx* c, float* ms) { B200_CHECK(c && ms, "b200_ctx_elapsed_ms"); B200_CUDA(cudaEventSynchronize(c->ev[1])); B200_CUDA(cudaEventElapsedTime(ms, c->ev[0], c->ev[1])); return 0; }
B200_API long long b200_ctx_kernel_launches(b200_ctx* c) { return c ? c->launches : 0; }

B200_API int b200_ctx_set_profiling(b200_ctx* c, int on) { B200_CHECK(c, "b200_ctx_set_profiling"); c->profiling = on != 0; return 0; }

B200_API int b200_ctx_get_kernel_ms_n(b200_ctx* c, float* ms, int* counts, int n)
{
  B200_CHECK(c && ms && counts && n >= 1 && n <= B200_KF_COUNT, "b200_ctx_get_kernel_ms_n");
  B200_CUDA(cudaStreamSynchronize(c->stream));
  for (int i = 0; i < n; i++) { ms[i] = 0; counts[i] = 0; }
  for (auto& r : c->prof.recs) { float t = 0; cudaEventElapsedTime(&t, r.a, r.b); if (r.family < n) { ms[r.family] += t; counts[r.family]++; } c->prof.pool.push_back(r.a); c->prof.pool.push_back(r.b); }
  c->prof.recs.clear();
  return 0;
}
B200_API int b200_ctx_get_kernel_ms(b200_ctx* c, float ms[8], int counts[8]) { return b200_ctx_get_kernel_ms_n(c, ms, counts, 8); }

B200_API int b200_host_register(void* ptr, size_t bytes) { B200_CHECK(ptr && bytes, "b200_host_register"); if (int rc = ensure_device()) return rc; B200_CUDA(cudaHostRegister(ptr, bytes, cudaHostRegisterDefault)); return 0; }
B200_API int b200_host_unregister(void* ptr) { B200_CHECK(ptr, "b200_host_unregister"); B200_CUDA(cudaHostUnregister(ptr)); return 0; }

}
```

Before: 1130.

## Fuse ALF luma, chroma and CC-ALF into one tiled kernel with shared staging

Replaces the separate luma and chroma ALF kernels, previously run on two streams, with a single kernel over a 1D grid of 32x32 luma blocks. Each block stages the luma tile and both chroma tiles into shared memory with cp.async and preloads all per-CTU luma filter taps, pre-packed, into shared memory. Classification reads packed words, and CC-ALF reads luma from the shared tile instead of global memory. This removes one launch, the stream fork and join, and redundant global reads of luma for CC-ALF. In exchange it uses a larger shared-memory footprint per block, which may limit occupancy, and runs chroma serially within the block on only 128 threads.

```diff
diff --git a/vvdec_b200/csrc/api.cu b/vvdec_b200/csrc/api.cu
--- a/vvdec_b200/csrc/api.cu
+++ b/vvdec_b200/csrc/api.cu
@@ -273,8 +273,7 @@
   if (int rc = up(T->ccCoeff[0], n0, L.cc[0])) return rc;
   if (int rc = up(T->ccCoeff[1], n1, L.cc[1])) return rc;
   L.ctus = g_hw.misc[0].as<b200_alf_ctu>();
-  StreamSet ss(s);
-  if (int rc = launch_alf(L, ss)) return rc;
+  if (int rc = launch_alf(L, s)) return rc;
   if (int rc = download_planes(g, dst, L.dst, s)) return rc;
   B200_CUDA(cudaStreamSynchronize(s));
   return 0;
diff --git a/vvdec_b200/csrc/common.cuh b/vvdec_b200/csrc/common.cuh
--- a/vvdec_b200/csrc/common.cuh
+++ b/vvdec_b200/csrc/common.cuh
@@ -125,7 +125,7 @@
   b200_geom geom; DevPlanes src, dst; const b200_alf_ctu* ctus;
   const int16_t *lumaCoeff, *lumaClip, *chromaCoeff, *chromaClip, *cc[2];
 };
-int launch_alf(const AlfLaunch& L, StreamSet& ss, KProf* prof = nullptr);
+int launch_alf(const AlfLaunch& L, cudaStream_t s, KProf* prof = nullptr);
 
 constexpr int B200_MAX_SLOTS = 32;
 struct McLaunch {
diff --git a/vvdec_b200/csrc/k5_alf.cu b/vvdec_b200/csrc/k5_alf.cu
--- a/vvdec_b200/csrc/k5_alf.cu
+++ b/vvdec_b200/csrc/k5_alf.cu
@@ -2,20 +2,36 @@
 
 namespace b200 {
 
+constexpr int NT = 256;
 constexpr int TB = 32;
 constexpr int HALO = 4;
 constexpr int TS = TB + 2 * HALO;
 constexpr int TSW = 44;
+constexpr int CB = TB / 2;
+constexpr int CTR = CB + 4;
+constexpr int CTC = CB + 8;
+constexpr int CSW = 28;
 
 struct AlfParams {
   const int16_t* src[3]; int16_t* dst[3]; int stride[3];
   int W, H, bitDepth, ctuSize, ctuLog2, ctusW;
+  int chroma;
+  int nby, nBlocks;
   int vecOk;
   int vecOkC;
   const b200_alf_ctu* ctus;
   const int16_t *lumaCoeff, *lumaClip, *chromaCoeff, *chromaClip, *cc0, *cc1;
 };
 
+struct AlfSmem {
+  __align__(16) int16_t y[TS][TSW];
+  __align__(16) int16_t c[2][CTR][CSW];
+  uint2 tap[4 * 25][12];
+  int cf[2][12];
+  int ccf[2][7];
+  uint8_t cls[64];
+};
+
 __device__ __forceinline__ void cp_async8(void* smemDst, const void* gmemSrc)
 {
   const unsigned d = (unsigned)__cvta_generic_to_shared(smemDst);
@@ -32,171 +48,194 @@
 }
 
 __device__ __forceinline__ int clipd(int c, int ref, int a, int b) { return clip3(-c, c, a - ref) + clip3(-c, c, b - ref); }
-
-__global__ void __launch_bounds__(256) alf_luma_kernel(const AlfParams P)
-{
-  __shared__ __align__(16) int16_t t[TS][TSW];
-  __shared__ uint16_t s_cls[64];
-  const int bx0 = blockIdx.x * TB, by0 = blockIdx.y * TB;
+__device__ __forceinline__ void unpack4(const uint2 u, int* d) { d[0] = (int)(int16_t)(u.x & 0xffff); d[1] = (int)u.x >> 16; d[2] = (int)(int16_t)(u.y & 0xffff); d[3] = (int)u.y >> 16; }
+__device__ __forceinline__ void lds12(const int16_t* p, int* v)
+{
+#pragma unroll
+  for (int j = 0; j < 3; j++) unpack4(*reinterpret_cast<const uint2*>(p + 4 * j), v + 4 * j);
+}
+__device__ __forceinline__ uint2 pack4(const int* o) { return make_uint2((unsigned)(o[0] & 0xffff) | ((unsigned)o[1] << 16), (unsigned)(o[2] & 0xffff) | ((unsigned)o[3] << 16)); }
+
+struct AlfBlk {
+  int bx0, by0; b200_alf_ctu cp;
+  bool lumaOn, stY, stC[2];
+};
+__device__ __forceinline__ AlfBlk alf_blk(const AlfParams& P, int b)
+{
+  AlfBlk B;
+  const int col = b / P.nby;
+  B.bx0 = col * TB; B.by0 = (b - col * P.nby) * TB;
+  B.cp = P.ctus[(B.by0 >> P.ctuLog2) * P.ctusW + (B.bx0 >> P.ctuLog2)];
+  B.lumaOn = B.cp.enable[0] & 1;
+  const bool cc = P.chroma && (B.cp.ccIdx[0] || B.cp.ccIdx[1]);
+  B.stY = B.lumaOn || cc;
+  for (int k = 0; k < 2; k++) B.stC[k] = P.chroma && ((B.cp.enable[1 + k] & 1) || B.cp.ccIdx[k]);
+  return B;
+}
+
+template <int ROWS, int COLS, int SW>
+__device__ __forceinline__ void stage_plane(int16_t* t, const int16_t* s, int stride, int gx0, int gy0, bool vec, const AlfExt& E)
+{
+  if (vec) {
+    for (int i = threadIdx.x; i < ROWS * (COLS / 4); i += NT) {
+      const int ty = i / (COLS / 4), c = i - ty * (COLS / 4);
+      cp_async8(t + ty * SW + c * 4, s + (size_t)(gy0 + ty) * stride + gx0 + c * 4);
+    }
+  } else {
+    for (int i = threadIdx.x; i < ROWS * COLS; i += NT) {
+      const int ty = i / COLS, tx = i - ty * COLS;
+      int gx = gx0 + tx, gy = gy0 + ty;
+      if (E.f) alf_map(E, gx, gy);
+      else { gx = min(max(gx, 0), E.W - 1); gy = min(max(gy, 0), E.H - 1); }
+      t[ty * SW + tx] = s[(size_t)gy * stride + gx];
+    }
+  }
+}
+
+__device__ __forceinline__ void stage_block(const AlfParams& P, const AlfBlk& B, AlfSmem& S)
+{
+  const int clipF = B.cp.enable[0] & ~1;
+  if (B.stY) {
+    AlfExt E; E.x0 = (B.bx0 >> P.ctuLog2) << P.ctuLog2; E.y0 = (B.by0 >> P.ctuLog2) << P.ctuLog2; E.x1 = min(E.x0 + P.ctuSize, P.W) - 1; E.y1 = min(E.y0 + P.ctuSize, P.H) - 1;
+    E.W = P.W; E.H = P.H; E.f = clipF; E.pm = 0;
+    const bool vec = !clipF && P.vecOk && B.bx0 >= HALO && B.bx0 + TB + HALO <= P.W && B.by0 >= HALO && B.by0 + TB + HALO <= P.H;
+    stage_plane<TS, TS, TSW>(&S.y[0][0], P.src[0], P.stride[0], B.bx0 - HALO, B.by0 - HALO, vec, E);
+  }
+  const int pw = P.W >> 1, ph = P.H >> 1, cx0 = B.bx0 >> 1, cy0 = B.by0 >> 1, l2cs = P.ctuLog2 - 1;
+  for (int k = 0; k < 2; k++) {
+    if (!B.stC[k]) continue;
+    AlfExt E; E.x0 = (cx0 >> l2cs) << l2cs; E.y0 = (cy0 >> l2cs) << l2cs; E.x1 = min(E.x0 + (1 << l2cs), pw) - 1; E.y1 = min(E.y0 + (1 << l2cs), ph) - 1;
+    E.W = pw; E.H = ph; E.f = clipF; E.pm = (B.cp.enable[1 + k] & B200_ALF_PAD_WIDE) ? 2 : 0;
+    const bool vec = !clipF && P.vecOkC && cx0 >= 4 && cx0 + CB + 4 <= pw && cy0 >= 2 && cy0 + CB + 2 <= ph;
+    stage_plane<CTR, CTC, CSW>(&S.c[k][0][0], P.src[1 + k], P.stride[1 + k], cx0 - 4, cy0 - 2, vec, E);
+  }
+}
+
+__device__ __forceinline__ void alf_classify(const AlfParams& P, const AlfBlk& B, AlfSmem& S)
+{
   const int tid = threadIdx.x;
-  const b200_alf_ctu cp = P.ctus[(by0 >> P.ctuLog2) * P.ctusW + (bx0 >> P.ctuLog2)];
-  const int stride = P.stride[0];
-  const int bw = min(TB, P.W - bx0), bh = min(TB, P.H - by0);
-
-  if (!(cp.enable[0] & 1)) {
-    for (int i = tid; i < bh * (bw >> 2); i += 256) {
-      const int y = i / (bw >> 2), x = (i - y * (bw >> 2)) * 4;
-      *reinterpret_cast<uint2*>(P.dst[0] + (size_t)(by0 + y) * stride + bx0 + x) = *reinterpret_cast<const uint2*>(P.src[0] + (size_t)(by0 + y) * stride + bx0 + x);
-    }
-    return;
-  }
-
-  const int clipF = cp.enable[0] & ~1;
-  if (clipF) {
-    AlfExt E; E.x0 = (bx0 >> P.ctuLog2) << P.ctuLog2; E.y0 = (by0 >> P.ctuLog2) << P.ctuLog2; E.x1 = min(E.x0 + P.ctuSize, P.W) - 1; E.y1 = min(E.y0 + P.ctuSize, P.H) - 1;
-    E.W = P.W; E.H = P.H; E.f = clipF; E.pm = 0;
-    for (int i = tid; i < TS * TS; i += 256) {
-      const int ty = i / TS, tx = i - ty * TS;
-      int gx = bx0 + tx - HALO, gy = by0 + ty - HALO;
-      alf_map(E, gx, gy);
-      t[ty][tx] = P.src[0][(size_t)gy * stride + gx];
-    }
-  } else if (P.vecOk && bx0 >= HALO && bx0 + TB + HALO <= P.W && by0 >= HALO && by0 + TB + HALO <= P.H) {
-    const int16_t* s0 = P.src[0] + (size_t)(by0 - HALO) * stride + bx0 - HALO;
-    for (int i = tid; i < TS * (TS / 4); i += 256) {
-      const int ty = i / (TS / 4), c = i - ty * (TS / 4);
-      cp_async8(&t[ty][c * 4], reinterpret_cast<const uint2*>(s0 + (size_t)ty * stride) + c);
-    }
-    asm volatile("cp.async.wait_all;\n" ::: "memory");
-  } else {
-    for (int i = tid; i < TS * TS; i += 256) {
-      const int ty = i / TS, tx = i - ty * TS;
-      const int gx = min(max(bx0 + tx - HALO, 0), P.W - 1), gy = min(max(by0 + ty - HALO, 0), P.H - 1);
-      t[ty][tx] = P.src[0][(size_t)gy * stride + gx];
-    }
-  }
-  __syncthreads();
-
+  const int16_t (*t)[TSW] = S.y;
   const int vbH = P.ctuSize, vbPos = P.ctuSize - 4;
-
-  {
-    const int b = tid >> 2, r = tid & 3;
-    const int bxi = b & 7, byi = b >> 3;
-    const int y0 = by0 + byi * 4, x0l = bxi * 4;
-    const bool aboveVb = (y0 & (vbH - 1)) == vbPos - 4, belowVb = (y0 & (vbH - 1)) == vbPos;
-    int sV = 0, sH = 0, sD0 = 0, sD1 = 0;
-    const bool skip = (aboveVb && r == 3) || (belowVb && r == 0);
-    if (!skip) {
-      const int gy = y0 - 2 + 2 * r;
-      const int ly = byi * 4 - 2 + 2 * r + HALO;
-      int up = -1, dn2 = 2;
-      if (gy > 0 && (gy & (vbH - 1)) == vbPos - 2) dn2 = 1;
-      else if (gy > 0 && (gy & (vbH - 1)) == vbPos) up = 0;
-#pragma unroll
-      for (int c = 0; c < 4; c++) {
-        const int lx = x0l - 2 + 2 * c + HALO;
-        const int a = t[ly][lx] << 1, bb = t[ly + 1][lx + 1] << 1;
-        sV  += abs(a - t[ly + up][lx] - t[ly + 1][lx])          + abs(bb - t[ly][lx + 1] - t[ly + dn2][lx + 1]);
-        sH  += abs(a - t[ly][lx + 1] - t[ly][lx - 1])           + abs(bb - t[ly + 1][lx + 2] - t[ly + 1][lx]);
-        sD0 += abs(a - t[ly + up][lx - 1] - t[ly + 1][lx + 1])  + abs(bb - t[ly][lx] - t[ly + dn2][lx + 2]);
-        sD1 += abs(a - t[ly + 1][lx - 1] - t[ly + up][lx + 1])  + abs(bb - t[ly + dn2][lx] - t[ly][lx + 2]);
-      }
-    }
-#pragma unroll
-    for (int m = 1; m < 4; m <<= 1) {
-      sV += __shfl_xor_sync(0xffffffffu, sV, m); sH += __shfl_xor_sync(0xffffffffu, sH, m);
-      sD0 += __shfl_xor_sync(0xffffffffu, sD0, m); sD1 += __shfl_xor_sync(0xffffffffu, sD1, m);
-    }
-    if (r == 0) {
-      const int shift = P.bitDepth + 4;
-      const int act = clip3(0, 15, ((sV + sH) * ((aboveVb || belowVb) ? 96 : 64)) >> shift);
-      const unsigned long long TH = 0x4333333332222210ull;
-      int classIdx = (int)((TH >> (4 * act)) & 15);
-      int hv1, hv0, d1, d0, dirHV, dirD;
-      if (sV > sH) { hv1 = sV; hv0 = sH; dirHV = 1; } else { hv1 = sH; hv0 = sV; dirHV = 3; }
-      if (sD0 > sD1) { d1 = sD0; d0 = sD1; dirD = 0; } else { d1 = sD1; d0 = sD0; dirD = 2; }
-      int hvd1, hvd0, mainDir, secDir;
-      if ((unsigned)d1 * (unsigned)hv0 > (unsigned)hv1 * (unsigned)d0) { hvd1 = d1; hvd0 = d0; mainDir = dirD; secDir = dirHV; }
-      else { hvd1 = hv1; hvd0 = hv0; mainDir = dirHV; secDir = dirD; }
-      int strength = 0;
-      if (hvd1 > 2 * hvd0) strength = 1;
-      if (hvd1 * 2 > 9 * hvd0) strength = 2;
-      if (strength) classIdx += (((mainDir & 1) << 1) + strength) * 5;
-      const unsigned TT = 0x31322010u;
-      const int tr = (TT >> (4 * (mainDir * 2 + (secDir >> 1)))) & 15;
-      s_cls[b] = (uint16_t)(classIdx | (tr << 8));
-    }
-  }
-  __syncthreads();
-
-  {
-    const int ry = tid >> 3, rx = (tid & 7) * 4;
-    if (ry >= bh || rx >= bw) return;
-    const uint16_t k = s_cls[(ry >> 2) * 8 + (rx >> 2)];
-    const int off = (k & 0xff) * 13 + (k >> 8) * 13 * 25 + cp.lumaSet * 4 * 25 * 13;
-    const int16_t* f = P.lumaCoeff + off; const int16_t* c = P.lumaClip + off;
-    int fc[12], cc[12];
-#pragma unroll
-    for (int i = 0; i < 12; i++) { fc[i] = __ldg(f + i); cc[i] = __ldg(c + i); }
-    const int gy = by0 + ry, yVb = gy & (vbH - 1);
-    int lim = 3;
-    if (yVb < vbPos && yVb >= vbPos - 4) lim = vbPos - 1 - yVb;
-    else if (yVb >= vbPos && yVb <= vbPos + 3) lim = yVb - vbPos;
-    const bool nearVb = yVb == vbPos - 1 || yVb == vbPos;
-    const int r1 = min(1, lim), r2 = min(2, lim), r3 = min(3, lim);
-    const int ly = ry + HALO;
-    const int pmax = (1 << P.bitDepth) - 1;
-    const int lx0 = rx + HALO;
-    int out[4];
-    bool wide = P.bitDepth > 12;
-#pragma unroll
-    for (int i = 0; i < 12; i++) wide |= fc[i] != (int)(int8_t)fc[i];
-    if (!wide) {
-      const uint32_t* R0 = reinterpret_cast<const uint32_t*>(&t[ly][0]) + (lx0 >> 1);
-      const uint32_t* P1 = reinterpret_cast<const uint32_t*>(&t[ly + r1][0]) + (lx0 >> 1); const uint32_t* M1 = reinterpret_cast<const uint32_t*>(&t[ly - r1][0]) + (lx0 >> 1);
-      const uint32_t* P2 = reinterpret_cast<const uint32_t*>(&t[ly + r2][0]) + (lx0 >> 1); const uint32_t* M2 = reinterpret_cast<const uint32_t*>(&t[ly - r2][0]) + (lx0 >> 1);
-      const uint32_t* P3 = reinterpret_cast<const uint32_t*>(&t[ly + r3][0]) + (lx0 >> 1); const uint32_t* M3 = reinterpret_cast<const uint32_t*>(&t[ly - r3][0]) + (lx0 >> 1);
-      uint32_t r0w[6], p1w[4], m1w[4], p2w[4], m2w[4], p3w[2], m3w[2];
-#pragma unroll
-      for (int k = 0; k < 6; k++) r0w[k] = R0[k - 2];
-#pragma unroll
-      for (int k = 0; k < 4; k++) { p1w[k] = P1[k - 1]; m1w[k] = M1[k - 1]; p2w[k] = P2[k - 1]; m2w[k] = M2[k - 1]; }
-#pragma unroll
-      for (int k = 0; k < 2; k++) { p3w[k] = P3[k]; m3w[k] = M3[k]; }
-      uint32_t r0s[5], p1s[3], m1s[3], p2s[3], m2s[3];
-#pragma unroll
-      for (int k = 0; k < 5; k++) r0s[k] = __byte_perm(r0w[k], r0w[k + 1], 0x5432);
-#pragma unroll
-      for (int k = 0; k < 3; k++) {
-        p1s[k] = __byte_perm(p1w[k], p1w[k + 1], 0x5432); m1s[k] = __byte_perm(m1w[k], m1w[k + 1], 0x5432);
-        p2s[k] = __byte_perm(p2w[k], p2w[k + 1], 0x5432); m2s[k] = __byte_perm(m2w[k], m2w[k + 1], 0x5432);
-      }
-      int accLo[2] = {0, 0}, accHi[2] = {0, 0};
-      uint32_t ncur[2] = {__vneg2(r0w[2]), __vneg2(r0w[3])};
+  const int b = tid >> 2, r = tid & 3;
+  const int bxi = b & 7, byi = b >> 3;
+  const int y0 = B.by0 + byi * 4, x0l = bxi * 4;
+  const bool aboveVb = (y0 & (vbH - 1)) == vbPos - 4, belowVb = (y0 & (vbH - 1)) == vbPos;
+  int sV = 0, sH = 0, sD0 = 0, sD1 = 0;
+  const bool skip = (aboveVb && r == 3) || (belowVb && r == 0);
+  if (!skip) {
+    const int gy = y0 - 2 + 2 * r;
+    const int ly = byi * 4 - 2 + 2 * r + HALO;
+    uint32_t w[4][6];
+#pragma unroll
+    for (int rr = 0; rr < 4; rr++)
+#pragma unroll
+      for (int j = 0; j < 3; j++) { const uint2 u = *reinterpret_cast<const uint2*>(&t[ly - 1 + rr][x0l + 4 * j]); w[rr][2 * j] = u.x; w[rr][2 * j + 1] = u.y; }
+    const bool upSame = gy > 0 && (gy & (vbH - 1)) == vbPos, dnNear = gy > 0 && (gy & (vbH - 1)) == vbPos - 2;
+    uint32_t wu[6], wd[6];
+#pragma unroll
+    for (int k = 0; k < 6; k++) { wu[k] = upSame ? w[1][k] : w[0][k]; wd[k] = dnNear ? w[2][k] : w[3][k]; }
+#define SMP(row, col) (((col) & 1) ? (int)(row)[(col) >> 1] >> 16 : (int)(int16_t)((row)[(col) >> 1] & 0xffff))
+#pragma unroll
+    for (int c = 0; c < 4; c++) {
+      const int lx = 2 + 2 * c;
+      const int a = SMP(w[1], lx) << 1, bb = SMP(w[2], lx + 1) << 1;
+      sV  += abs(a - SMP(wu, lx) - SMP(w[2], lx))            + abs(bb - SMP(w[1], lx + 1) - SMP(wd, lx + 1));
+      sH  += abs(a - SMP(w[1], lx + 1) - SMP(w[1], lx - 1))  + abs(bb - SMP(w[2], lx + 2) - SMP(w[2], lx));
+      sD0 += abs(a - SMP(wu, lx - 1) - SMP(w[2], lx + 1))    + abs(bb - SMP(w[1], lx) - SMP(wd, lx + 2));
+      sD1 += abs(a - SMP(w[2], lx - 1) - SMP(wu, lx + 1))    + abs(bb - SMP(wd, lx) - SMP(w[1], lx + 2));
+    }
+#undef SMP
+  }
+#pragma unroll
+  for (int m = 1; m < 4; m <<= 1) {
+    sV += __shfl_xor_sync(0xffffffffu, sV, m); sH += __shfl_xor_sync(0xffffffffu, sH, m);
+    sD0 += __shfl_xor_sync(0xffffffffu, sD0, m); sD1 += __shfl_xor_sync(0xffffffffu, sD1, m);
+  }
+  const int shift = P.bitDepth + 4;
+  const int act = clip3(0, 15, ((sV + sH) * ((aboveVb || belowVb) ? 96 : 64)) >> shift);
+  const unsigned long long TH = 0x4333333332222210ull;
+  int classIdx = (int)((TH >> (4 * act)) & 15);
+  int hv1, hv0, d1, d0, dirHV, dirD;
+  if (sV > sH) { hv1 = sV; hv0 = sH; dirHV = 1; } else { hv1 = sH; hv0 = sV; dirHV = 3; }
+  if (sD0 > sD1) { d1 = sD0; d0 = sD1; dirD = 0; } else { d1 = sD1; d0 = sD0; dirD = 2; }
+  int hvd1, hvd0, mainDir, secDir;
+  if ((unsigned)d1 * (unsigned)hv0 > (unsigned)hv1 * (unsigned)d0) { hvd1 = d1; hvd0 = d0; mainDir = dirD; secDir = dirHV; }
+  else { hvd1 = hv1; hvd0 = hv0; mainDir = dirHV; secDir = dirD; }
+  int strength = 0;
+  if (hvd1 > 2 * hvd0) strength = 1;
+  if (hvd1 * 2 > 9 * hvd0) strength = 2;
+  if (strength) classIdx += (((mainDir & 1) << 1) + strength) * 5;
+  const unsigned TT = 0x31322010u;
+  const int tr = (TT >> (4 * (mainDir * 2 + (secDir >> 1)))) & 15;
+  if (r == 0) S.cls[b] = (uint8_t)(tr * 25 + classIdx);
+}
+
+__device__ __forceinline__ void alf_filter_luma(const AlfParams& P, const AlfBlk& B, const AlfSmem& S, bool wide)
+{
+  const int tid = threadIdx.x;
+  const int16_t (*t)[TSW] = S.y;
+  const int ry = tid >> 3, rx = (tid & 7) * 4;
+  if (ry >= P.H - B.by0 || rx >= P.W - B.bx0) return;
+  const int vbH = P.ctuSize, vbPos = P.ctuSize - 4;
+  const int blk4 = (ry >> 2) * 8 + (rx >> 2);
+  const int k = S.cls[blk4];
+  const int gy = B.by0 + ry, yVb = gy & (vbH - 1);
+  int lim = 3;
+  if (yVb < vbPos && yVb >= vbPos - 4) lim = vbPos - 1 - yVb;
+  else if (yVb >= vbPos && yVb <= vbPos + 3) lim = yVb - vbPos;
+  const bool nearVb = yVb == vbPos - 1 || yVb == vbPos;
+  const int r1 = min(1, lim), r2 = min(2, lim), r3 = min(3, lim);
+  const int ly = ry + HALO;
+  const int pmax = (1 << P.bitDepth) - 1;
+  const int lx0 = rx + HALO;
+  int out[4];
+  if (!wide) {
+    const uint2* tp = S.tap[k];
+    const uint32_t* R0 = reinterpret_cast<const uint32_t*>(&t[ly][0]) + (lx0 >> 1);
+    const uint32_t* P1 = reinterpret_cast<const uint32_t*>(&t[ly + r1][0]) + (lx0 >> 1); const uint32_t* M1 = reinterpret_cast<const uint32_t*>(&t[ly - r1][0]) + (lx0 >> 1);
+    const uint32_t* P2 = reinterpret_cast<const uint32_t*>(&t[ly + r2][0]) + (lx0 >> 1); const uint32_t* M2 = reinterpret_cast<const uint32_t*>(&t[ly - r2][0]) + (lx0 >> 1);
+    const uint32_t* P3 = reinterpret_cast<const uint32_t*>(&t[ly + r3][0]) + (lx0 >> 1); const uint32_t* M3 = reinterpret_cast<const uint32_t*>(&t[ly - r3][0]) + (lx0 >> 1);
+    uint32_t r0w[6], p1w[4], m1w[4], p2w[4], m2w[4], p3w[2], m3w[2];
+#pragma unroll
+    for (int k = 0; k < 6; k++) r0w[k] = R0[k - 2];
+#pragma unroll
+    for (int k = 0; k < 4; k++) { p1w[k] = P1[k - 1]; m1w[k] = M1[k - 1]; p2w[k] = P2[k - 1]; m2w[k] = M2[k - 1]; }
+#pragma unroll
+    for (int k = 0; k < 2; k++) { p3w[k] = P3[k]; m3w[k] = M3[k]; }
+    uint32_t r0s[5], p1s[3], m1s[3], p2s[3], m2s[3];
+#pragma unroll
+    for (int k = 0; k < 5; k++) r0s[k] = __byte_perm(r0w[k], r0w[k + 1], 0x5432);
+#pragma unroll
+    for (int k = 0; k < 3; k++) {
+      p1s[k] = __byte_perm(p1w[k], p1w[k + 1], 0x5432); m1s[k] = __byte_perm(m1w[k], m1w[k + 1], 0x5432);
+      p2s[k] = __byte_perm(p2w[k], p2w[k + 1], 0x5432); m2s[k] = __byte_perm(m2w[k], m2w[k + 1], 0x5432);
+    }
+    int accLo[2] = {0, 0}, accHi[2] = {0, 0};
+    uint32_t ncur[2] = {__vneg2(r0w[2]), __vneg2(r0w[3])};
 #define R0P(j) (((j) & 1) ? r0s[((j) + 3) >> 1] : r0w[((j) + 4) >> 1])
 #define P1P(j) (((j) & 1) ? p1s[((j) + 1) >> 1] : p1w[((j) + 2) >> 1])
 #define M1P(j) (((j) & 1) ? m1s[((j) + 1) >> 1] : m1w[((j) + 2) >> 1])
 #define P2P(j) (((j) & 1) ? p2s[((j) + 1) >> 1] : p2w[((j) + 2) >> 1])
 #define M2P(j) (((j) & 1) ? m2s[((j) + 1) >> 1] : m2w[((j) + 2) >> 1])
 #define ALF_TAP(n, A0, B0, A1, B1) { \
-        const uint32_t cp = (uint32_t)cc[n] * 0x10001u, cn = __vneg2(cp); const int kl = fc[n] & 0xff, kh = kl << 8; \
-        uint32_t d0 = __vmins2(__vmaxs2(__vadd2(A0, ncur[0]), cn), cp), e0 = __vmins2(__vmaxs2(__vadd2(B0, ncur[0]), cn), cp); \
-        uint32_t d1 = __vmins2(__vmaxs2(__vadd2(A1, ncur[1]), cn), cp), e1 = __vmins2(__vmaxs2(__vadd2(B1, ncur[1]), cn), cp); \
-        d0 = __vadd2(d0, e0); d1 = __vadd2(d1, e1); \
-        accLo[0] = __dp2a_lo((int)d0, kl, accLo[0]); accHi[0] = __dp2a_lo((int)d0, kh, accHi[0]); \
-        accLo[1] = __dp2a_lo((int)d1, kl, accLo[1]); accHi[1] = __dp2a_lo((int)d1, kh, accHi[1]); }
-      ALF_TAP(0,  p3w[0],  m3w[0],  p3w[1],  m3w[1])
-      ALF_TAP(1,  P2P(1),  M2P(-1), P2P(3),  M2P(1))
-      ALF_TAP(2,  P2P(0),  M2P(0),  P2P(2),  M2P(2))
-      ALF_TAP(3,  P2P(-1), M2P(1),  P2P(1),  M2P(3))
-      ALF_TAP(4,  P1P(2),  M1P(-2), P1P(4),  M1P(0))
-      ALF_TAP(5,  P1P(1),  M1P(-1), P1P(3),  M1P(1))
-      ALF_TAP(6,  P1P(0),  M1P(0),  P1P(2),  M1P(2))
-      ALF_TAP(7,  P1P(-1), M1P(1),  P1P(1),  M1P(3))
-      ALF_TAP(8,  P1P(-2), M1P(2),  P1P(0),  M1P(4))
-      ALF_TAP(9,  R0P(3),  R0P(-3), R0P(5),  R0P(-1))
-      ALF_TAP(10, R0P(2),  R0P(-2), R0P(4),  R0P(0))
-      ALF_TAP(11, R0P(1),  R0P(-1), R0P(3),  R0P(1))
+      const uint2 tw = tp[n]; const uint32_t cp = tw.x, cn = __vneg2(cp); const int kw = (int)tw.y; \
+      uint32_t d0 = __vmins2(__vmaxs2(__vadd2(A0, ncur[0]), cn), cp), e0 = __vmins2(__vmaxs2(__vadd2(B0, ncur[0]), cn), cp); \
+      uint32_t d1 = __vmins2(__vmaxs2(__vadd2(A1, ncur[1]), cn), cp), e1 = __vmins2(__vmaxs2(__vadd2(B1, ncur[1]), cn), cp); \
+      d0 = __vadd2(d0, e0); d1 = __vadd2(d1, e1); \
+      accLo[0] = __dp2a_lo((int)d0, kw, accLo[0]); accHi[0] = __dp2a_hi((int)d0, kw, accHi[0]); \
+      accLo[1] = __dp2a_lo((int)d1, kw, accLo[1]); accHi[1] = __dp2a_hi((int)d1, kw, accHi[1]); }
+    ALF_TAP(0,  p3w[0],  m3w[0],  p3w[1],  m3w[1])
+    ALF_TAP(1,  P2P(1),  M2P(-1), P2P(3),  M2P(1))
+    ALF_TAP(2,  P2P(0),  M2P(0),  P2P(2),  M2P(2))
+    ALF_TAP(3,  P2P(-1), M2P(1),  P2P(1),  M2P(3))
+    ALF_TAP(4,  P1P(2),  M1P(-2), P1P(4),  M1P(0))
+    ALF_TAP(5,  P1P(1),  M1P(-1), P1P(3),  M1P(1))
+    ALF_TAP(6,  P1P(0),  M1P(0),  P1P(2),  M1P(2))
+    ALF_TAP(7,  P1P(-1), M1P(1),  P1P(1),  M1P(3))
+    ALF_TAP(8,  P1P(-2), M1P(2),  P1P(0),  M1P(4))
+    ALF_TAP(9,  R0P(3),  R0P(-3), R0P(5),  R0P(-1))
+    ALF_TAP(10, R0P(2),  R0P(-2), R0P(4),  R0P(0))
+    ALF_TAP(11, R0P(1),  R0P(-1), R0P(3),  R0P(1))
 #undef ALF_TAP
 #undef R0P
 #undef P1P
@@ -204,12 +243,17 @@
 #undef P2P
 #undef M2P
 #pragma unroll
-      for (int q = 0; q < 2; q++) {
-        const int c0 = (int)(int16_t)(r0w[2 + q] & 0xffff), c1 = (int)r0w[2 + q] >> 16;
-        const int s0 = nearVb ? (accLo[q] + 512) >> 10 : (accLo[q] + 64) >> 7, s1 = nearVb ? (accHi[q] + 512) >> 10 : (accHi[q] + 64) >> 7;
-        out[2 * q] = clip3(0, pmax, s0 + c0); out[2 * q + 1] = clip3(0, pmax, s1 + c1);
-      }
-    } else {
+    for (int q = 0; q < 2; q++) {
+      const int c0 = (int)(int16_t)(r0w[2 + q] & 0xffff), c1 = (int)r0w[2 + q] >> 16;
+      const int s0 = nearVb ? (accLo[q] + 512) >> 10 : (accLo[q] + 64) >> 7, s1 = nearVb ? (accHi[q] + 512) >> 10 : (accHi[q] + 64) >> 7;
+      out[2 * q] = clip3(0, pmax, s0 + c0); out[2 * q + 1] = clip3(0, pmax, s1 + c1);
+    }
+  } else {
+    const int off = k * 13 + B.cp.lumaSet * 4 * 25 * 13;
+    const int16_t* f = P.lumaCoeff + off; const int16_t* c = P.lumaClip + off;
+    int fc[12], cc[12];
+#pragma unroll
+    for (int i = 0; i < 12; i++) { fc[i] = __ldg(f + i); cc[i] = __ldg(c + i); }
     int r0[10], p1[8], m1[8], p2[6], m2[6], p3[4], m3[4];
 #pragma unroll
     for (int k = 0; k < 10; k++) r0[k] = t[ly][lx0 - 3 + k];
@@ -238,154 +282,147 @@
       sum = nearVb ? (sum + 512) >> 10 : (sum + 64) >> 7;
       out[i] = clip3(0, pmax, sum + cur);
     }
-    }
-    uint2 o;
-    o.x = (unsigned)(out[0] & 0xffff) | ((unsigned)out[1] << 16);
-    o.y = (unsigned)(out[2] & 0xffff) | ((unsigned)out[3] << 16);
-    *reinterpret_cast<uint2*>(P.dst[0] + (size_t)gy * stride + bx0 + rx) = o;
-  }
-}
-
-__device__ __forceinline__ void unpack4(const uint2 u, int* d) { d[0] = (int)(int16_t)(u.x & 0xffff); d[1] = (int)u.x >> 16; d[2] = (int)(int16_t)(u.y & 0xffff); d[3] = (int)u.y >> 16; }
-
-__global__ void __launch_bounds__(256) alf_chroma_kernel(const AlfParams P)
-{
-  const int c = 1 + blockIdx.z;
-  const int pw = P.W >> 1, ph = P.H >> 1;
-  const int x = (blockIdx.x * 32 + threadIdx.x) * 4, y = blockIdx.y * 8 + threadIdx.y;
-  if (x >= pw || y >= ph) return;
-  const int l2cs = P.ctuLog2 - 1, cs = 1 << l2cs;
-  const b200_alf_ctu cp = P.ctus[(y >> l2cs) * P.ctusW + (x >> l2cs)];
+  }
+  *reinterpret_cast<uint2*>(P.dst[0] + (size_t)gy * P.stride[0] + B.bx0 + rx) = pack4(out);
+}
+
+__device__ __forceinline__ void alf_filter_chroma(const AlfParams& P, const AlfBlk& B, const AlfSmem& S)
+{
+  const int tid = threadIdx.x;
+  const int k = tid >> 6, c = 1 + k, yl = (tid >> 2) & 15, xl = (tid & 3) * 4;
+  const int x = (B.bx0 >> 1) + xl, y = (B.by0 >> 1) + yl;
+  if (x >= (P.W >> 1) || y >= (P.H >> 1)) return;
+  const bool staged = k ? B.stC[1] : B.stC[0];
+  const int en = k ? B.cp.enable[2] : B.cp.enable[1], ccIdx = k ? B.cp.ccIdx[1] : B.cp.ccIdx[0];
   const int stride = P.stride[c];
-  const int16_t* s = P.src[c];
   const int pmax = (1 << P.bitDepth) - 1;
-  const int clipF = cp.enable[0] & ~1;
-  const bool inner = P.vecOkC && x >= 4 && x + 8 <= pw && !clipF;
   int out[4];
-  AlfExt E; E.x0 = (x >> l2cs) << l2cs; E.y0 = (y >> l2cs) << l2cs; E.x1 = min(E.x0 + cs, pw) - 1; E.y1 = min(E.y0 + cs, ph) - 1; E.W = pw; E.H = ph; E.f = clipF;
-  E.pm = (cp.enable[c] & B200_ALF_PAD_WIDE) ? 2 : 0;
-  auto rowp = [&](int yy) { return s + (size_t)min(max(yy, 0), ph - 1) * stride; };
-  auto at = [&](int xx, int yy) { if (clipF) { alf_map(E, xx, yy); return (int)s[(size_t)yy * stride + xx]; } return (int)rowp(yy)[min(max(xx, 0), pw - 1)]; };
-  if (cp.enable[c] & 1) {
-    const int16_t* f = P.chromaCoeff + cp.chromaAlt[c - 1] * 7; const int16_t* cl = P.chromaClip + cp.chromaAlt[c - 1] * 7;
-    int fc[6], cc[6];
-#pragma unroll
-    for (int i = 0; i < 6; i++) { fc[i] = __ldg(f + i); cc[i] = __ldg(cl + i); }
-    const int vbH = cs, vbPos = cs - 2, yVb = y & (vbH - 1);
-    int lim = 2;
-    if (yVb < vbPos && yVb >= vbPos - 2) lim = vbPos - 1 - yVb;
-    else if (yVb >= vbPos && yVb <= vbPos + 1) lim = yVb - vbPos;
-    const bool nearVb = yVb == vbPos - 1 || yVb == vbPos;
-    const int r1 = min(1, lim), r2 = min(2, lim);
-    int r0[8], p1[6], m1[6], p2[4], m2[4];
-    if (inner) {
-      int t[4];
-      const int16_t* q = rowp(y) + x;
-      unpack4(__ldg(reinterpret_cast<const uint2*>(q - 4)), t); r0[0] = t[2]; r0[1] = t[3];
-      unpack4(__ldg(reinterpret_cast<const uint2*>(q)), r0 + 2);
-      unpack4(__ldg(reinterpret_cast<const uint2*>(q + 4)), t); r0[6] = t[0]; r0[7] = t[1];
-      q = rowp(y + r1) + x; p1[0] = q[-1]; unpack4(__ldg(reinterpret_cast<const uint2*>(q)), p1 + 1); p1[5] = q[4];
-      q = rowp(y - r1) + x; m1[0] = q[-1]; unpack4(__ldg(reinterpret_cast<const uint2*>(q)), m1 + 1); m1[5] = q[4];
-      unpack4(__ldg(reinterpret_cast<const uint2*>(rowp(y + r2) + x)), p2);
-      unpack4(__ldg(reinterpret_cast<const uint2*>(rowp(y - r2) + x)), m2);
+  if (!staged) {
+    unpack4(*reinterpret_cast<const uint2*>(P.src[c] + (size_t)y * stride + x), out);
+  } else {
+    const int16_t (*tc)[CSW] = S.c[k];
+    const int ty = yl + 2, tx = xl + 4;
+    if (en & 1) {
+      int fc[6], cc[6];
+#pragma unroll
+      for (int i = 0; i < 6; i++) { fc[i] = S.cf[k][i]; cc[i] = S.cf[k][6 + i]; }
+      const int cs = P.ctuSize >> 1, vbPos = cs - 2, yVb = y & (cs - 1);
+      int lim = 2;
+      if (yVb < vbPos && yVb >= vbPos - 2) lim = vbPos - 1 - yVb;
+      else if (yVb >= vbPos && yVb <= vbPos + 1) lim = yVb - vbPos;
+      const bool nearVb = yVb == vbPos - 1 || yVb == vbPos;
+      const int r1 = min(1, lim), r2 = min(2, lim);
+      int r0[12], p1[12], m1[12], p2[4], m2[4];
+      lds12(&tc[ty][tx - 4], r0); lds12(&tc[ty + r1][tx - 4], p1); lds12(&tc[ty - r1][tx - 4], m1);
+      unpack4(*reinterpret_cast<const uint2*>(&tc[ty + r2][tx]), p2); unpack4(*reinterpret_cast<const uint2*>(&tc[ty - r2][tx]), m2);
+#pragma unroll
+      for (int i = 0; i < 4; i++) {
+        const int cur = r0[i + 4];
+        int sum = 0;
+        sum += fc[0] * clipd(cc[0], cur, p2[i],     m2[i]);
+        sum += fc[1] * clipd(cc[1], cur, p1[i + 5], m1[i + 3]);
+        sum += fc[2] * clipd(cc[2], cur, p1[i + 4], m1[i + 4]);
+        sum += fc[3] * clipd(cc[3], cur, p1[i + 3], m1[i + 5]);
+        sum += fc[4] * clipd(cc[4], cur, r0[i + 6], r0[i + 2]);
+        sum += fc[5] * clipd(cc[5], cur, r0[i + 5], r0[i + 3]);
+        sum = nearVb ? (sum + 512) >> 10 : (sum + 64) >> 7;
+        out[i] = clip3(0, pmax, sum + cur);
+      }
     } else {
-#pragma unroll
-      for (int k = 0; k < 8; k++) r0[k] = at(x - 2 + k, y);
-#pragma unroll
-      for (int k = 0; k < 6; k++) { p1[k] = at(x - 1 + k, y + r1); m1[k] = at(x - 1 + k, y - r1); }
-#pragma unroll
-      for (int k = 0; k < 4; k++) { p2[k] = at(x + k, y + r2); m2[k] = at(x + k, y - r2); }
-    }
-#pragma unroll
-    for (int i = 0; i < 4; i++) {
-      const int cur = r0[i + 2];
-      int sum = 0;
-      sum += fc[0] * clipd(cc[0], cur, p2[i],     m2[i]);
-      sum += fc[1] * clipd(cc[1], cur, p1[i + 2], m1[i]);
-      sum += fc[2] * clipd(cc[2], cur, p1[i + 1], m1[i + 1]);
-      sum += fc[3] * clipd(cc[3], cur, p1[i],     m1[i + 2]);
-      sum += fc[4] * clipd(cc[4], cur, r0[i + 4], r0[i]);
-      sum += fc[5] * clipd(cc[5], cur, r0[i + 3], r0[i + 1]);
-      sum = nearVb ? (sum + 512) >> 10 : (sum + 64) >> 7;
-      out[i] = clip3(0, pmax, sum + cur);
-    }
-  } else {
-    unpack4(*reinterpret_cast<const uint2*>(s + (size_t)y * stride + x), out);
-  }
-  const int ccIdx = cp.ccIdx[c - 1];
-  if (ccIdx) {
-    const int16_t* f = (c == 1 ? P.cc0 : P.cc1) + (ccIdx - 1) * 7;
-    int fc[7];
-#pragma unroll
-    for (int i = 0; i < 7; i++) fc[i] = __ldg(f + i);
-    const int16_t* L = P.src[0]; const int ls = P.stride[0];
-    const int ly = y << 1, pos = ly & (P.ctuSize - 1), vbPos = P.ctuSize - 4;
-    int o1 = 1, o2 = -1, o3 = 2;
-    if (pos == vbPos - 2 || pos == vbPos + 1) o3 = 1;
-    else if (pos == vbPos - 1 || pos == vbPos) o1 = o2 = o3 = 0;
-    AlfExt EL; EL.x0 = E.x0 << 1; EL.y0 = E.y0 << 1; EL.x1 = min(EL.x0 + P.ctuSize, P.W) - 1; EL.y1 = min(EL.y0 + P.ctuSize, P.H) - 1; EL.W = P.W; EL.H = P.H; EL.f = clipF; EL.pm = 0;
-    auto lrow = [&](int yy) { return L + (size_t)min(max(yy, 0), P.H - 1) * ls; };
-    auto lat = [&](int xx, int yy) { if (clipF) { alf_map(EL, xx, yy); return (int)L[(size_t)yy * ls + xx]; } return (int)lrow(yy)[min(max(xx, 0), P.W - 1)]; };
-    const int half = (1 << P.bitDepth) >> 1;
-    int a[9], bb[9], up[4], dn[4];
-    if (inner) {
-      int t[4];
-      const int16_t* q = lrow(ly) + 2 * x;
-      a[0] = q[-1]; unpack4(__ldg(reinterpret_cast<const uint2*>(q)), a + 1); unpack4(__ldg(reinterpret_cast<const uint2*>(q + 4)), a + 5);
-      q = lrow(ly + o1) + 2 * x;
-      bb[0] = q[-1]; unpack4(__ldg(reinterpret_cast<const uint2*>(q)), bb + 1); unpack4(__ldg(reinterpret_cast<const uint2*>(q + 4)), bb + 5);
-      q = lrow(ly + o2) + 2 * x;
-      unpack4(__ldg(reinterpret_cast<const uint2*>(q)), t); up[0] = t[0]; up[1] = t[2]; unpack4(__ldg(reinterpret_cast<const uint2*>(q + 4)), t); up[2] = t[0]; up[3] = t[2];
-      q = lrow(ly + o3) + 2 * x;
-      unpack4(__ldg(reinterpret_cast<const uint2*>(q)), t); dn[0] = t[0]; dn[1] = t[2]; unpack4(__ldg(reinterpret_cast<const uint2*>(q + 4)), t); dn[2] = t[0]; dn[3] = t[2];
-    } else {
-#pragma unroll
-      for (int k = 0; k < 9; k++) { a[k] = lat(2 * x - 1 + k, ly); bb[k] = lat(2 * x - 1 + k, ly + o1); }
-#pragma unroll
-      for (int i = 0; i < 4; i++) { up[i] = lat(2 * (x + i), ly + o2); dn[i] = lat(2 * (x + i), ly + o3); }
-    }
-#pragma unroll
-    for (int i = 0; i < 4; i++) {
-      const int cur = a[2 * i + 1];
-      int sum = fc[0] * (up[i] - cur) + fc[1] * (a[2 * i] - cur) + fc[2] * (a[2 * i + 2] - cur)
-              + fc[3] * (bb[2 * i] - cur) + fc[4] * (bb[2 * i + 1] - cur) + fc[5] * (bb[2 * i + 2] - cur)
-              + fc[6] * (dn[i] - cur);
-      sum = (sum + 64) >> 7;
-      sum = clip3(0, pmax, sum + half) - half;
-      out[i] = clip3(0, pmax, sum + out[i]);
-    }
-  }
-  uint2 o;
-  o.x = (unsigned)(out[0] & 0xffff) | ((unsigned)out[1] << 16);
-  o.y = (unsigned)(out[2] & 0xffff) | ((unsigned)out[3] << 16);
-  *reinterpret_cast<uint2*>(P.dst[c] + (size_t)y * stride + x) = o;
-}
-
-int launch_alf(const AlfLaunch& L, StreamSet& ss, KProf* prof)
-{
-  cudaStream_t s = ss.main;
+      unpack4(*reinterpret_cast<const uint2*>(P.src[c] + (size_t)y * stride + x), out);
+    }
+    if (ccIdx) {
+      int fc[7];
+#pragma unroll
+      for (int i = 0; i < 7; i++) fc[i] = S.ccf[k][i];
+      const int16_t (*t)[TSW] = S.y;
+      const int pos = (y << 1) & (P.ctuSize - 1), vbPos = P.ctuSize - 4;
+      int o1 = 1, o2 = -1, o3 = 2;
+      if (pos == vbPos - 2 || pos == vbPos + 1) o3 = 1;
+      else if (pos == vbPos - 1 || pos == vbPos) o1 = o2 = o3 = 0;
+      const int lty = 2 * yl + HALO, ltx = 2 * xl + HALO;
+      const int half = (1 << P.bitDepth) >> 1;
+      int a[12], bb[12], up[8], dn[8];
+      lds12(&t[lty][ltx - 4], a); lds12(&t[lty + o1][ltx - 4], bb);
+#pragma unroll
+      for (int j = 0; j < 2; j++) { unpack4(*reinterpret_cast<const uint2*>(&t[lty + o2][ltx + 4 * j]), up + 4 * j); unpack4(*reinterpret_cast<const uint2*>(&t[lty + o3][ltx + 4 * j]), dn + 4 * j); }
+#pragma unroll
+      for (int i = 0; i < 4; i++) {
+        const int cur = a[2 * i + 4];
+        int sum = fc[0] * (up[2 * i] - cur) + fc[1] * (a[2 * i + 3] - cur) + fc[2] * (a[2 * i + 5] - cur)
+                + fc[3] * (bb[2 * i + 3] - cur) + fc[4] * (bb[2 * i + 4] - cur) + fc[5] * (bb[2 * i + 5] - cur)
+                + fc[6] * (dn[2 * i] - cur);
+        sum = (sum + 64) >> 7;
+        sum = clip3(0, pmax, sum + half) - half;
+        out[i] = clip3(0, pmax, sum + out[i]);
+      }
+    }
+  }
+  *reinterpret_cast<uint2*>(P.dst[c] + (size_t)y * stride + x) = pack4(out);
+}
+
+__device__ __forceinline__ void alf_copy_luma(const AlfParams& P, const AlfBlk& B)
+{
+  const int ry = threadIdx.x >> 3, rx = (threadIdx.x & 7) * 4;
+  if (ry >= P.H - B.by0 || rx >= P.W - B.bx0) return;
+  const size_t o = (size_t)(B.by0 + ry) * P.stride[0] + B.bx0 + rx;
+  *reinterpret_cast<uint2*>(P.dst[0] + o) = *reinterpret_cast<const uint2*>(P.src[0] + o);
+}
+
+__device__ __forceinline__ int alf_load_filters(const AlfParams& P, const AlfBlk& B, AlfSmem& S)
+{
+  const int tid = threadIdx.x;
+  int wide = 0;
+  if (B.lumaOn) {
+    const int16_t* f = P.lumaCoeff + B.cp.lumaSet * 4 * 25 * 13; const int16_t* c = P.lumaClip + B.cp.lumaSet * 4 * 25 * 13;
+    for (int i = tid; i < 4 * 25 * 12; i += NT) {
+      const int fl = i / 12, j = i - fl * 12;
+      const int v = __ldg(f + fl * 13 + j), cl = __ldg(c + fl * 13 + j);
+      wide |= v != (int)(int8_t)v;
+      S.tap[fl][j] = make_uint2((uint32_t)cl * 0x10001u, ((uint32_t)v & 0xff) * 0x01000001u);
+    }
+  }
+  if (P.chroma && tid < 24) {
+    const int k = tid / 12, j = tid - k * 12;
+    if ((k ? B.cp.enable[2] : B.cp.enable[1]) & 1) { const int o = (k ? B.cp.chromaAlt[1] : B.cp.chromaAlt[0]) * 7 + (j < 6 ? j : j - 6); S.cf[k][j] = __ldg((j < 6 ? P.chromaCoeff : P.chromaClip) + o); }
+  } else if (P.chroma && tid >= 32 && tid < 32 + 14) {
+    const int k = (tid - 32) / 7, j = tid - 32 - k * 7;
+    const int idx = k ? B.cp.ccIdx[1] : B.cp.ccIdx[0];
+    if (idx) S.ccf[k][j] = __ldg((k ? P.cc1 : P.cc0) + (idx - 1) * 7 + j);
+  }
+  return wide;
+}
+
+__global__ void __launch_bounds__(NT, 3) alf_kernel(const AlfParams P)
+{
+  __shared__ AlfSmem S;
+  const AlfBlk B = alf_blk(P, blockIdx.x);
+  stage_block(P, B, S);
+  int wide = alf_load_filters(P, B, S);
+  asm volatile("cp.async.wait_all;\n" ::: "memory");
+  wide = __syncthreads_or(wide) || P.bitDepth > 12;
+  if (B.lumaOn) alf_classify(P, B, S);
+  __syncthreads();
+  if (B.lumaOn) alf_filter_luma(P, B, S, wide); else alf_copy_luma(P, B);
+  if (P.chroma && threadIdx.x < 128) alf_filter_chroma(P, B, S);
+}
+
+int launch_alf(const AlfLaunch& L, cudaStream_t s, KProf* prof)
+{
   AlfParams P;
   for (int c = 0; c < 3; c++) { P.src[c] = L.src.p[c]; P.dst[c] = L.dst.p[c]; P.stride[c] = L.src.stride[c]; }
   P.W = L.geom.width; P.H = L.geom.height; P.bitDepth = L.geom.bitDepth; P.ctuSize = L.geom.ctuSize;
   P.ctuLog2 = P.ctuSize == 128 ? 7 : P.ctuSize == 64 ? 6 : 5; P.ctusW = (P.W + P.ctuSize - 1) / P.ctuSize;
+  P.chroma = L.geom.chromaFormat == 1;
+  P.nby = (P.H + TB - 1) / TB; P.nBlocks = P.nby * ((P.W + TB - 1) / TB);
   P.ctus = L.ctus; P.lumaCoeff = L.lumaCoeff; P.lumaClip = L.lumaClip; P.chromaCoeff = L.chromaCoeff; P.chromaClip = L.chromaClip;
   P.cc0 = L.cc[0]; P.cc1 = L.cc[1];
   P.vecOk = (P.stride[0] & 3) == 0 && (reinterpret_cast<uintptr_t>(P.src[0]) & 7) == 0;
-  P.vecOkC = P.vecOk && (P.stride[1] & 3) == 0 && (P.stride[2] & 3) == 0 && (reinterpret_cast<uintptr_t>(P.src[1]) & 7) == 0 && (reinterpret_cast<uintptr_t>(P.src[2]) & 7) == 0;
-  dim3 grdL((P.W + TB - 1) / TB, (P.H + TB - 1) / TB);
-  if (L.geom.chromaFormat == 1) {
-    cudaStream_t sc = ss.pick(0);
-    dim3 blk(32, 8), grd(((P.W >> 1) / 4 + 31) / 32, ((P.H >> 1) + 7) / 8, 2);
-    if (prof) prof->begin(B200_KF_ALF_CHROMA, sc);
-    alf_chroma_kernel<<<grd, blk, 0, sc>>>(P);
-    B200_CUDA(cudaGetLastError());
-    if (prof) prof->end(B200_KF_ALF_CHROMA, sc);
-  }
+  P.vecOkC = P.chroma && (P.stride[1] & 3) == 0 && (P.stride[2] & 3) == 0 && (reinterpret_cast<uintptr_t>(P.src[1]) & 7) == 0 && (reinterpret_cast<uintptr_t>(P.src[2]) & 7) == 0;
   if (prof) prof->begin(B200_KF_ALF_LUMA, s);
-  alf_luma_kernel<<<grdL, 256, 0, s>>>(P);
+  alf_kernel<<<P.nBlocks, NT, 0, s>>>(P);
   B200_CUDA(cudaGetLastError());
   if (prof) prof->end(B200_KF_ALF_LUMA, s);
-  ss.join();
   return 0;
 }
 
diff --git a/vvdec_b200/csrc/picture.cu b/vvdec_b200/csrc/picture.cu
--- a/vvdec_b200/csrc/picture.cu
+++ b/vvdec_b200/csrc/picture.cu
@@ -347,8 +347,8 @@
   if (A.flags & B200_PIC_ALF) {
     AlfLaunch L; L.geom = g; L.src = P; L.dst = c->planes(other); L.ctus = A.alf;
     L.lumaCoeff = A.lumaCoeff; L.lumaClip = A.lumaClip; L.chromaCoeff = A.chromaCoeff; L.chromaClip = A.chromaClip; L.cc[0] = A.cc[0]; L.cc[1] = A.cc[1];
-    if (int rc = launch_alf(L, c->ss, c->profiling ? &c->prof : nullptr)) return rc;
-    c->launches += g.chromaFormat ? 2 : 1;
+    if (int rc = launch_alf(L, s, c->profiling ? &c->prof : nullptr)) return rc;
+    c->launches += 1;
     std::swap(cur, other);
   }
   B200_CUDA(cudaEventRecord(A.done, s)); A.donePending = true;
```

Result: no change. 1132 (median of 6 runs) (+0.2%).
